# ngrabaskas/Torch-Automatic-Distributed-Neural-Network

Hardware: AMD Instinct MI355X
Metric: samples/sec whole-node ResNet-50 DP + GPT-2 PP at 1/2/4/8 MI355X; scaling eff (higher is better)
Workload: dtype bf16

## Files before the change

madnn/models/resnet.py:

```python
from __future__ import annotations

import os
from collections import namedtuple
from typing import List, Type

import torch
from torch import nn

from ..nn.conv import FusedConv2d
from ..nn.norm import FusedBatchNorm2d as BN
from ..nn.norm import FusedGlobalAvgPool2d, FusedMaxPool2d
from ..ops import (batch_norm_add_bn_relu, bn2_conv3_bn3_add_bn_relu, bn2_conv3_bn3_add_bn_relu_supported,
                   bn2_conv3_bn3_add_relu, bn2_conv3_bn3_supported, bn_relu_conv1x1,
                   bn_relu_conv1x1_epi_supported, bn_relu_conv3x3, bn_relu_conv3x3_supported, bn_relu_maxpool,
                   bn_relu_maxpool_supported, conv1x1_route, defer_res_mask)

_FORK_DS = os.environ.get("MADNN_FORK_DOWNSAMPLE", "1") != "0"
_DUAL_BN = os.environ.get("MADNN_DUAL_BN", "1") != "0"
_DS_SUB = os.environ.get("MADNN_DS_SUB", "1") != "0"


ROUTES = (IDENTITY_K9F, IDENTITY, DUAL_SUB, DUAL_K9F, DUAL, FORK_DS, PLAIN_DS) = (
    "identity+k9f", "identity", "dual+sub", "dual+k9f", "dual", "fork-ds", "plain-ds")
_Fused = namedtuple("_Fused", "bn1_conv2 bn2_conv3 bn3 dual")


def conv3x3(cin, cout, stride=1, groups=1, dilation=1):
    return FusedConv2d(cin, cout, 3, stride=stride, padding=dilation, groups=groups, bias=False, dilation=dilation)


def conv1x1(cin, cout, stride=1):
    return FusedConv2d(cin, cout, 1, stride=stride, bias=False)


class BasicBlock(nn.Module):
    expansion = 1

    def __init__(self, inplanes, planes, stride=1, downsample=None):
        super().__init__()
        self.conv1 = conv3x3(inplanes, planes, stride)
        self.bn1 = BN(planes)
        self.conv2 = conv3x3(planes, planes)
        self.bn2 = BN(planes)
        self.downsample = downsample

    def forward(self, x):
        idt = x if self.downsample is None else self.downsample(x)
        y, st = self.conv1(x, stats=True)
        out = self.bn1(y, relu=True, stats=st)
        y, st = self.conv2(out, stats=True)
        return self.bn2(y, residual=idt, relu=True, stats=st)


class Bottleneck(nn.Module):
    expansion = 4

    def __init__(self, inplanes, planes, stride=1, downsample=None):
        super().__init__()
        self.conv1 = conv1x1(inplanes, planes)
        self.bn1 = BN(planes)
        self.conv2 = conv3x3(planes, planes, stride)
        self.bn2 = BN(planes)
        self.conv3 = conv1x1(planes, planes * 4)
        self.bn3 = BN(planes * 4)
        self.downsample = downsample

    def forward(self, x):
        fused = self._fused()
        route = self._route(x, fused)
        ds = self.downsample
        if route in (IDENTITY_K9F, IDENTITY):
            y, st, side = self.conv1(x, stats=True, fork=True)
            if route == IDENTITY_K9F:
                defer_res_mask(side)
        elif route == PLAIN_DS:
            side = ds(x)
            y, st = self.conv1(x, stats=True)
        else:
            y, st, xf = self.conv1(x, stats=True, fork=2 if route == DUAL_SUB else True)
            if route == DUAL_K9F and not self._k9f_dual(y, xf):
                route = DUAL
            if route == FORK_DS:
                side = ds(xf)
            elif route == DUAL_SUB:
                side = ds[0].forward_subsampled(xf, stats=True)
            elif route == DUAL:
                side = ds[0](xf, stats=True)
        y1 = y
        y, st = self._bn1_conv2(y, st, fused)
        if route == IDENTITY_K9F and fused.bn2_conv3 and isinstance(y, torch.Tensor) and self.conv3._k9(y) \
                and bn2_conv3_bn3_supported(y, self.bn2, self.conv3.weight, self.bn3, side):
            return bn2_conv3_bn3_add_relu(y, self.bn2, self.conv3.weight, self.bn3, side, stats_in=st)
        if route == DUAL_K9F:
            if isinstance(y, torch.Tensor) and y.requires_grad \
                    and (y.shape, y.stride(), y.dtype) == (y1.shape, y1.stride(), y1.dtype):
                return bn2_conv3_bn3_add_bn_relu(y, self.bn2, self.conv3.weight, self.bn3, xf, ds[0].weight,
                                                 ds[1], stats_in=st)
            route, side = DUAL, ds[0](xf, stats=True)
        y, st = self._bn2_conv3(y, st, fused)
        if route in (DUAL_SUB, DUAL):
            return batch_norm_add_bn_relu(y, side[0], self.bn3, ds[1], st, side[1])
        return self.bn3(y, residual=side, relu=True, stats=st)

    def _fused(self) -> "_Fused":
        ds = self.downsample
        return _Fused(bn1_conv2=isinstance(self.bn1, BN) and isinstance(self.conv2, FusedConv2d),
                      bn2_conv3=isinstance(self.bn2, BN) and isinstance(self.conv3, FusedConv2d),
                      bn3=isinstance(self.bn3, BN),
                      dual=(isinstance(ds, nn.Sequential) and len(ds) == 2 and isinstance(ds[0], FusedConv2d)
                            and isinstance(ds[1], BN) and isinstance(self.bn3, BN)))

    def _dual_bn(self) -> bool:
        return _DUAL_BN and self._fused().dual

    def _route(self, x, fused: "_Fused") -> str:
        ds, tensor = self.downsample, isinstance(x, torch.Tensor)
        if ds is None:
            defer = (tensor and fused.bn3 and self.conv1._k9(x)
                     and conv1x1_route(x.size(1), self.conv1.weight.size(0))[1] == "k9")
            return IDENTITY_K9F if defer else IDENTITY
        if not _FORK_DS:
            return PLAIN_DS
        if not (_DUAL_BN and fused.dual):
            return FORK_DS
        if _DS_SUB and tensor and ds[0].subsampled_ok():
            return DUAL_SUB
        return DUAL_K9F if tensor and fused.bn2_conv3 and self.conv2.stride == (1, 1) else DUAL

    def _bn1_conv2(self, y, st, fused):
        if fused.bn1_conv2 and isinstance(y, torch.Tensor) and self.conv2._k13(y) \
                and bn_relu_conv3x3_supported(y, self.bn1, self.conv2.weight):
            return bn_relu_conv3x3(y, self.bn1, self.conv2.weight, stats_in=st, stats=True, checked=True)
        out = self.bn1(y, relu=True, stats=st)
        return self.conv2(out, stats=True)

    def _bn2_conv3(self, y, st, fused):
        if fused.bn2_conv3 and isinstance(y, torch.Tensor) and self.conv3._k9(y) \
                and bn_relu_conv1x1_epi_supported(y, self.bn2, self.conv3.weight):
            return bn_relu_conv1x1(y, self.bn2, self.conv3.weight, stats_in=st, stats=True, checked=True)
        out = self.bn2(y, relu=True, stats=st)
        return self.conv3(out, stats=True)

    def _k9f_dual(self, y1, xf) -> bool:
        ds = self.downsample
        return (isinstance(y1, torch.Tensor) and isinstance(xf, torch.Tensor) and self.conv3._k9(y1)
                and ds[0]._k9(xf) and bn2_conv3_bn3_add_bn_relu_supported(
                    y1, self.bn2, self.conv3.weight, self.bn3, xf, ds[0].weight, ds[1]))


class ResNet(nn.Module):
    def __init__(self, block: Type[nn.Module], layers: List[int], num_classes: int = 1000,
                 zero_init_residual: bool = True, width: int = 64):
        super().__init__()
        self.inplanes = width
        self.conv1 = FusedConv2d(3, width, 7, stride=2, padding=3, bias=False)
        self.bn1 = BN(width)
        self.maxpool = FusedMaxPool2d(3, stride=2, padding=1)
        self.layer1 = self._make_layer(block, width, layers[0])
        self.layer2 = self._make_layer(block, width * 2, layers[1], stride=2)
        self.layer3 = self._make_layer(block, width * 4, layers[2], stride=2)
        self.layer4 = self._make_layer(block, width * 8, layers[3], stride=2)
        self.avgpool = FusedGlobalAvgPool2d((1, 1))
        self.fc = nn.Linear(width * 8 * block.expansion, num_classes)
        for m in self.modules():
            if isinstance(m, nn.Conv2d):
                nn.init.kaiming_normal_(m.weight, mode="fan_out", nonlinearity="relu")
            elif isinstance(m, nn.BatchNorm2d):
                nn.init.ones_(m.weight)
                nn.init.zeros_(m.bias)
        if zero_init_residual:
            for m in self.modules():
                if isinstance(m, Bottleneck):
                    nn.init.zeros_(m.bn3.weight)
                elif isinstance(m, BasicBlock):
                    nn.init.zeros_(m.bn2.weight)

    def _make_layer(self, block, planes, blocks, stride=1):
        downsample = None
        if stride != 1 or self.inplanes != planes * block.expansion:
            downsample = nn.Sequential(conv1x1(self.inplanes, planes * block.expansion, stride),
                                       BN(planes * block.expansion))
        layers = [block(self.inplanes, planes, stride, downsample)]
        self.inplanes = planes * block.expansion
        layers += [block(self.inplanes, planes) for _ in range(1, blocks)]
        return nn.Sequential(*layers)

    def stem(self, x):
        y, st = self.conv1(x, stats=True)
        if isinstance(self.bn1, BN) and isinstance(self.maxpool, FusedMaxPool2d) \
                and bn_relu_maxpool_supported(y, self.bn1, self.maxpool):
            return bn_relu_maxpool(y, self.bn1, self.maxpool, st)
        return self.maxpool(self.bn1(y, relu=True, stats=st))

    def head(self, x):
        return self.fc(torch.flatten(self.avgpool(x), 1))

    def forward(self, x):
        x = self.layer4(self.layer3(self.layer2(self.layer1(self.stem(x)))))
        return self.head(x)

    def pipeline_layers(self):
        blocks = [b for layer in (self.layer1, self.layer2, self.layer3, self.layer4) for b in layer]
        return [_Bound(self, "stem"), *blocks, _Bound(self, "head")]


class _Bound(nn.Module):

    def __init__(self, model: nn.Module, method: str):
        super().__init__()
        self.parts = nn.ModuleDict({n: m for n, m in model.named_children()
                                    if n in {"stem": ("conv1", "bn1", "maxpool"),
                                             "head": ("avgpool", "fc")}[method]})
        object.__setattr__(self, "_model", model)
        self.method = method

    def forward(self, x):
        return getattr(self._model, self.method)(x)


def resnet18(num_classes: int = 1000, **kw) -> ResNet:
    return ResNet(BasicBlock, [2, 2, 2, 2], num_classes, **kw)


def resnet50(num_classes: int = 1000, **kw) -> ResNet:
    return ResNet(Bottleneck, [3, 4, 6, 3], num_classes, **kw)


def resnet101(num_classes: int = 1000, **kw) -> ResNet:
    return ResNet(Bottleneck, [3, 4, 23, 3], num_classes, **kw)
```

madnn/nn/conv.py:

```python
from __future__ import annotations

import os

import torch
from torch import nn

from .. import ops

_K9 = os.environ.get("MADNN_CONV1X1", "1") != "0"


class FusedConv2d(nn.Conv2d):
    def _k9(self, x: torch.Tensor) -> bool:
        return (_K9 and self.kernel_size == (1, 1) and self.stride == (1, 1) and self.dilation == (1, 1)
                and self.groups == 1 and self.bias is None and self.padding in ((0, 0), "valid")
                and ops.conv1x1_supported(x, self.weight))

    def _k13(self, x: torch.Tensor) -> bool:
        return (self.kernel_size == (3, 3) and self.stride == (1, 1) and self.padding == (1, 1)
                and self.dilation == (1, 1) and self.groups == 1 and self.bias is None
                and self.padding_mode == "zeros" and ops.conv3x3_supported(x, self.weight))

    def _k13s2(self, x: torch.Tensor) -> bool:
        return (self.kernel_size == (3, 3) and self.stride == (2, 2) and self.padding == (1, 1)
                and self.dilation == (1, 1) and self.groups == 1 and self.bias is None
                and self.padding_mode == "zeros" and ops.conv3x3_s2_supported(x, self.weight))

    def _k10(self, x: torch.Tensor) -> bool:
        return (self.kernel_size == (7, 7) and self.stride == (2, 2) and self.padding == (3, 3)
                and self.dilation == (1, 1) and self.groups == 1 and self.bias is None
                and ops.stem_supported(x, self.weight))

    def forward(self, x: torch.Tensor, stats: bool = False, fork: bool = False):
        if self._k9(x):
            return ops.conv1x1(x, self.weight, stats=stats, fork=fork)
        if not fork and self._k13(x):
            return ops.conv3x3(x, self.weight, stats=stats)
        if not fork and self._k13s2(x):
            return ops.conv3x3_s2(x, self.weight, stats=stats)
        if not fork and self._k10(x):
            return ops.stem_conv(x, self.weight, stats=stats)
        out = [super().forward(x)]
        if stats:
            out.append(None)
        if fork:
            out.append(x[:, :, ::2, ::2] if fork == 2 else x)
        return out[0] if len(out) == 1 else tuple(out)

    def subsampled_ok(self) -> bool:
        return (self.kernel_size == (1, 1) and self.stride == (2, 2) and self.padding in ((0, 0), "valid")
                and self.dilation == (1, 1) and self.groups == 1 and self.bias is None)

    def forward_subsampled(self, xs: torch.Tensor, stats: bool = False):
        if _K9 and ops.conv1x1_supported(xs, self.weight):
            return ops.conv1x1(xs, self.weight, stats=stats)
        y = torch.nn.functional.conv2d(xs, self.weight)
        return (y, None) if stats else y

    def extra_repr(self):
        k = {(1, 1): ", kernel=madnn.K9", (7, 7): ", kernel=madnn.K10",
             (3, 3): ", kernel=madnn.K13" if self.stride in ((1, 1), (2, 2)) else ""}.get(self.kernel_size, "")
        return super().extra_repr() + k
```

madnn/ops/__init__.py:

```python
from __future__ import annotations

import os
import threading
from pathlib import Path
from typing import Optional, Sequence

import torch
import torch.nn.functional as F

from . import reference

HERE = Path(__file__).resolve().parent
_KERNELS = HERE / "_madnn_kernels.so"
_lock = threading.Lock()
_loaded = {"kernels": False, "error": None}


def kernels_path() -> Path:
    return _KERNELS


class StaleKernelsError(RuntimeError):
    """The in-tree kernel library was built from different sources than the tree holds."""

# ... 714 lines not shown
        dout = _nhwc(dout.to(y.dtype))
        da, part = torch.ops.madnn.conv1x1_dgrad_bnb(dout, w, y, scale, shift)
        dw = _routed_conv1x1_wgrad(ctx.wgrad, dout, a, w)
        dy, dbw, dbb = torch.ops.madnn.bn_bwd_ext(da, y, bn_w, mean, invstd, scale, shift, part, True)
        need_bn = ctx.needs_input_grad[2] or ctx.needs_input_grad[3]
        return dy, dw, dbw if need_bn else None, dbb if need_bn else None, None, None, None


def bn_relu_conv1x1(y: torch.Tensor, bn, w: torch.Tensor, *, stats_in: Optional[torch.Tensor] = None,
                    stats: bool = False, checked: bool = False):
    if checked or bn_relu_conv1x1_epi_supported(y, bn, w):
        _need_native("bn_relu_conv1x1")
        return _with_stats(*_BNReluConv1x1EpiFn.apply(y, w, bn.weight, bn.bias, bn, stats_in, stats), stats)
    a = bn(y, relu=True, stats=stats_in) if _is_fused_bn(bn) else torch.relu(bn(y))
    if conv1x1_supported(a, w):
        return conv1x1(a, w, stats=stats)
    out = torch.nn.functional.conv2d(a, w.view(w.size(0), -1, 1, 1)) if a.dim() == 4 else torch.mm(
        a, w.reshape(w.size(0), -1).t())
    return (out, None) if stats else out


def bn_relu_conv1x1_epi_supported(y: torch.Tensor, bn, w: torch.Tensor) -> bool:
    return (_BN_DGRAD_EPI and isinstance(y, torch.Tensor) and _bn_trainable(bn)
            and conv1x1_supported(y, w) and bn_supported(y, bn.weight)
            and conv1x1_route(y.size(1), w.size(0))[1] == "k9")


def _k9f_head(y2, w3, bn2_w, bn2_b, bn2, stats_in):
    a2, mean2, invstd2, scale2, shift2, _ = _bn_fwd_train(y2, None, bn2_w, bn2_b, bn2, True, stats_in)
    y3, part = torch.ops.madnn.conv1x1_fwd(a2, w3, True)
    return a2, y3, part, (mean2, invstd2, scale2, shift2)


def _k9f_tail(ctx, da2, part, y2, bn2_w, bn2_stats, dw3, w3, dbw3, dbb3):
    dy2, dbw2, dbb2 = torch.ops.madnn.bn_bwd_ext(da2, y2, bn2_w, *bn2_stats, part, True)
    need2, need3 = (ctx.needs_input_grad[i] or ctx.needs_input_grad[i + 1] for i in (2, 4))
    return (dy2, dw3.to(w3.dtype).view(w3.shape), dbw2 if need2 else None, dbb2 if need2 else None,
            dbw3 if need3 else None, dbb3 if need3 else None)


class _BN2Conv3BN3Fn(torch.autograd.Function):

    @staticmethod
    def forward(ctx, y2, w3, bn2_w, bn2_b, bn3_w, bn3_b, idt, bn2, bn3, stats_in):
        a2, y3, part, bn2_stats = _k9f_head(y2, w3, bn2_w, bn2_b, bn2, stats_in)
        out, mean3, invstd3, scale3, shift3, mask = _bn_fwd_train(y3, idt, bn3_w, bn3_b, bn3, True, part)
        ctx.save_for_backward(y2, a2, w3, y3, mask, bn2_w, *bn2_stats, bn3_w, mean3, invstd3, scale3, shift3)
        return out

    @staticmethod
    def backward(ctx, dout):
        y2, a2, w3, y3, mask, bn2_w, *bn2_stats, bn3_w, mean3, invstd3, scale3, shift3 = ctx.saved_tensors
        dout = _like(dout, y3)
        coef, dbw3, dbb3 = torch.ops.madnn.bn_bwd_coef(dout, y3, mask, bn3_w, mean3, invstd3, scale3, shift3)
        da2, part, dw3 = torch.ops.madnn.bn3_conv3_bwd(dout, y3, mask, coef, w3, a2, y2, *bn2_stats[2:],
                                                       w3.dtype == torch.bfloat16)
        grads = _k9f_tail(ctx, da2, part, y2, bn2_w, bn2_stats, dw3, w3, dbw3, dbb3)
        dres = dout.view_as(dout)
        _attach(dres, "_madnn_resmask", mask)
        return (*grads, dres, None, None, None)


_BN3_CONV3_FUSED = os.environ.get("MADNN_BN3_CONV3_FUSED", "1") != "0"


def _k9f_supported(y2: torch.Tensor, bn2, w3: torch.Tensor, bn3, other: torch.Tensor) -> bool:
    return (_BN3_CONV3_FUSED and isinstance(y2, torch.Tensor) and isinstance(other, torch.Tensor)
            and bn_relu_conv1x1_epi_supported(y2, bn2, w3) and native_available()
            and bool(torch.ops.madnn.bn3_conv3_bwd_supported(y2.size(1), w3.size(0)))
            and conv1x1_route(y2.size(1), w3.size(0))[0] == "k9" and _bn_trainable(bn3)
            and bn3.weight.numel() == w3.size(0) and y2.requires_grad and torch.is_grad_enabled()
            and other.dtype == y2.dtype and other.dim() == y2.dim() and other.size(0) == y2.size(0)
            and other.shape[2:] == y2.shape[2:])


def bn2_conv3_bn3_supported(y2: torch.Tensor, bn2, w3: torch.Tensor, bn3, idt: torch.Tensor) -> bool:
    return (DEFER_RES_MASK and _k9f_supported(y2, bn2, w3, bn3, idt) and _res_mask_deferred(idt)
            and idt.size(1) == w3.size(0) and bn_supported(idt, bn3.weight))


def bn2_conv3_bn3_add_relu(y2: torch.Tensor, bn2, w3: torch.Tensor, bn3, idt: torch.Tensor,
                           stats_in: Optional[torch.Tensor] = None) -> torch.Tensor:
    _need_native("bn2_conv3_bn3_add_relu")
    return _BN2Conv3BN3Fn.apply(y2, w3, bn2.weight, bn2.bias, bn3.weight, bn3.bias, idt, bn2, bn3, stats_in)


class _BN2Conv3BN3DualFn(torch.autograd.Function):

    @staticmethod
    def forward(ctx, y2, w3, bn2_w, bn2_b, bn3_w, bn3_b, xf, w_ds, bnd_w, bnd_b, bn2, bn3, bn_ds, stats_in):
        a2, y3, part, bn2_stats = _k9f_head(y2, w3, bn2_w, bn2_b, bn2, stats_in)
        yd, part_d = torch.ops.madnn.conv1x1_fwd(xf, w_ds, True)
        out, mask, mean3, invstd3, _, _, mean_d, invstd_d, _, _ = torch.ops.madnn.bn_fwd_dual(
            y3, yd, bn3_w, bn3_b, bn3.running_mean, bn3.running_var, bn3.num_batches_tracked, float(bn3.momentum),
            float(bn3.eps), part, bnd_w, bnd_b, bn_ds.running_mean, bn_ds.running_var, bn_ds.num_batches_tracked,
            float(bn_ds.momentum), float(bn_ds.eps), part_d)
        ctx.save_for_backward(y2, a2, w3, y3, xf, w_ds, yd, mask, bn2_w, *bn2_stats, bn3_w, mean3, invstd3, bnd_w,
                              mean_d, invstd_d)
        return out

    @staticmethod
    def backward(ctx, dout):
        (y2, a2, w3, y3, xf, w_ds, yd, mask, bn2_w, *bn2_stats, bn3_w, mean3, invstd3, bnd_w, mean_d,
         invstd_d) = ctx.saved_tensors
        dout = _like(dout, y3)
        coef, dbw3, dbb3, dbwd, dbbd = torch.ops.madnn.bn_bwd_dual_coef(dout, y3, yd, mask, bn3_w, mean3, invstd3,
                                                                        bnd_w, mean_d, invstd_d)
        da2, part, dw3 = torch.ops.madnn.bn3_conv3_bwd(dout, y3, mask, coef[:3], w3, a2, y2, *bn2_stats[2:],
                                                       w3.dtype == torch.bfloat16)
        dxf, _, dwd = torch.ops.madnn.bn3_conv3_bwd(dout, yd, mask, coef[3:], w_ds, xf, None, None, None,
                                                    w_ds.dtype == torch.bfloat16)
        grads = _k9f_tail(ctx, da2, part, y2, bn2_w, bn2_stats, dw3, w3, dbw3, dbb3)
        needd = ctx.needs_input_grad[8] or ctx.needs_input_grad[9]
        return (*grads, dxf, dwd.to(w_ds.dtype).view(w_ds.shape), dbwd if needd else None,
                dbbd if needd else None, None, None, None, None)


_BN3_CONV3_DUAL = os.environ.get("MADNN_BN3_CONV3_DUAL", "1") != "0"


def bn2_conv3_bn3_add_bn_relu_supported(y2: torch.Tensor, bn2, w3: torch.Tensor, bn3, xf: torch.Tensor,
                                        w_ds: torch.Tensor, bn_ds) -> bool:
    return (_BN3_CONV3_DUAL and _k9f_supported(y2, bn2, w3, bn3, xf) and conv1x1_supported(xf, w_ds)
            and xf.size(1) == y2.size(1) and w_ds.size(0) == w3.size(0) and _bn_trainable(bn_ds)
            and bn_ds.weight.numel() == w3.size(0))


def bn2_conv3_bn3_add_bn_relu(y2: torch.Tensor, bn2, w3: torch.Tensor, bn3, xf: torch.Tensor, w_ds: torch.Tensor,
                              bn_ds, stats_in: Optional[torch.Tensor] = None) -> torch.Tensor:
    _need_native("bn2_conv3_bn3_add_bn_relu")
    return _BN2Conv3BN3DualFn.apply(y2, w3, bn2.weight, bn2.bias, bn3.weight, bn3.bias, xf, w_ds, bn_ds.weight,
                                    bn_ds.bias, bn2, bn3, bn_ds, stats_in)


class _BNReluMaxPoolFn(torch.autograd.Function):

    @staticmethod
    def forward(ctx, y, bn_w, bn_b, bn, stats_in, p):
        mean, invstd, scale, shift = torch.ops.madnn.bn_coef(y, bn_w, bn_b, bn.running_mean, bn.running_var,
                                                             bn.num_batches_tracked, float(bn.momentum),
                                                             float(bn.eps), stats_in)
        out, arg = torch.ops.madnn.pool_bn_fwd(y, scale, shift, int(p))
        ctx.save_for_backward(y, arg, bn_w, mean, invstd, scale, shift)
        ctx.p = int(p)
        return out

    @staticmethod
    def backward(ctx, dp):
        y, arg, bn_w, mean, invstd, scale, shift = ctx.saved_tensors
        dy, dw, db = torch.ops.madnn.pool_bn_bwd(dp, arg, y, bn_w, mean, invstd, scale, shift, ctx.p)
        return dy, dw, db, None, None, None


def bn_relu_maxpool_supported(y: torch.Tensor, bn, pool) -> bool:
    return (_POOL_BN and isinstance(y, torch.Tensor) and y.device.type == "cuda" and y.dtype == torch.bfloat16 and y.dim() == 4
            and y.is_contiguous(memory_format=torch.channels_last) and _bn_trainable(bn)
            and _pair(pool.kernel_size) == (3, 3) and _pair(pool.stride) == (2, 2)
            and _pair(pool.padding) in ((1, 1), (0, 0)) and _pair(pool.dilation) == (1, 1)
            and not pool.ceil_mode and not pool.return_indices
            and y.size(1) % 8 == 0 and 256 % (y.size(1) // 8) == 0 and y.numel() < 2 ** 31)


def bn_relu_maxpool(y: torch.Tensor, bn, pool, stats_in: Optional[torch.Tensor] = None):
    if bn_relu_maxpool_supported(y, bn, pool):
        _need_native("bn_relu_maxpool")
        p = pool.padding if isinstance(pool.padding, int) else pool.padding[0]
        return _BNReluMaxPoolFn.apply(y, bn.weight, bn.bias, bn, stats_in, p)
    a = bn(y, relu=True, stats=stats_in) if _is_fused_bn(bn) else torch.relu(bn(y))
    return pool(a)


_POOL_BN = os.environ.get("MADNN_POOL_BN", "1") != "0"


_K13 = os.environ.get("MADNN_CONV3X3", "1") != "0"
_K13_WGRAD = os.environ.get("MADNN_CONV3X3_WGRAD", "auto")


def _k13_halo_ok(W: int) -> bool:
    rb = 2 * 32
    rpi = 1024 // rb
    cap = ((255 // W) * W + 4 * W + rpi - 1) // rpi * rpi
    return max(cap * rb + rb + 2 * 64 * rb, 32 * 1024) <= 80 * 1024


def _k13_operands_ok(x: torch.Tensor, w: torch.Tensor) -> bool:
    if not _K13 or x.device.type != "cuda" or x.dtype != torch.bfloat16 or w.dtype != torch.bfloat16:
        return False
    if x.dim() != 4 or not x.is_contiguous(memory_format=torch.channels_last) or x.numel() == 0:
        return False
    if w.dim() != 4 or tuple(w.shape[1:]) != (x.size(1), 3, 3):
        return False
    return x.size(1) % 64 == 0 and w.size(0) % 64 == 0


def conv3x3_supported(x: torch.Tensor, w: torch.Tensor) -> bool:
    return _k13_operands_ok(x, w) and _k13_halo_ok(x.size(3))


def _flip3x3(w: torch.Tensor) -> torch.Tensor:
    return w.flip(2, 3).transpose(0, 1).contiguous(memory_format=torch.channels_last)


def _conv3x3_wgrad(dy: torch.Tensor, x: torch.Tensor, w: torch.Tensor) -> torch.Tensor:
    k13 = lambda: torch.ops.madnn.conv3x3_wgrad(dy, x, w.dtype == torch.bfloat16)
    lib = lambda: torch.ops.aten.convolution_backward(
        dy, x, w, None, (1, 1), (1, 1), (1, 1), False, (0, 0), 1, (False, True, False))[1]
    if _K13_WGRAD == "k13":
        dw = k13()
    elif _K13_WGRAD == "miopen" or (_K13_WGRAD == "wide" and x.size(3) < 48):
        dw = lib()
    elif _K13_WGRAD == "wide":
        dw = k13()
    else:
        dw = tuned_wgrad(("conv3x3",) + tuple(x.shape) + (w.size(0),), lib, k13)
    return _like(dw, w)


class _Conv3x3Fn(torch.autograd.Function):

    @staticmethod
    def forward(ctx, x, w, stats):
        y, part = torch.ops.madnn.conv3x3_fwd(x, _nhwc(w), bool(stats))
        ctx.save_for_backward(x, w)
        ctx.mark_non_differentiable(part)
        return y, part

    @staticmethod
    def backward(ctx, dy, _dpart):
        x, w = ctx.saved_tensors
        dy = _nhwc(dy.to(x.dtype))
        dx = dw = None
        if ctx.needs_input_grad[0]:
            dx = torch.ops.madnn.conv3x3_fwd(dy, _flip3x3(w), False)[0]
        if ctx.needs_input_grad[1]:
            dw = _conv3x3_wgrad(dy, x, w)
        return dx, dw, None


class _BNReluConv3x3Fn(torch.autograd.Function):

    @staticmethod
    def forward(ctx, y, w, bn_w, bn_b, bn, stats_in, want_stats):
        a, mean, invstd, scale, shift, _ = _bn_fwd_train(y, None, bn_w, bn_b, bn, True, stats_in)
        out, part = torch.ops.madnn.conv3x3_fwd(a, _nhwc(w), bool(want_stats))
        ctx.save_for_backward(y, a, w, bn_w, mean, invstd, scale, shift)
        ctx.mark_non_differentiable(part)
        return out, part

    @staticmethod
    def backward(ctx, dout, _dpart):
        y, a, w, bn_w, mean, invstd, scale, shift = ctx.saved_tensors
        dout = _nhwc(dout.to(y.dtype))
        da, part = torch.ops.madnn.conv3x3_fwd_bnb(dout, _flip3x3(w), y, scale, shift)
        dw = _conv3x3_wgrad(dout, a, w)
        dy, dbw, dbb = torch.ops.madnn.bn_bwd_ext(da, y, bn_w, mean, invstd, scale, shift, part, True)
        need_bn = ctx.needs_input_grad[2] or ctx.needs_input_grad[3]
        return dy, dw, dbw if need_bn else None, dbb if need_bn else None, None, None, None


def bn_relu_conv3x3_supported(y: torch.Tensor, bn, w: torch.Tensor) -> bool:
    return (_BN_DGRAD_EPI and isinstance(y, torch.Tensor) and _bn_trainable(bn) and conv3x3_supported(y, w)
            and y.size(1) == w.size(1) and bn_supported(y, bn.weight))


def bn_relu_conv3x3(y: torch.Tensor, bn, w: torch.Tensor, *, stats_in: Optional[torch.Tensor] = None,
                    stats: bool = False, checked: bool = False):
    if checked or bn_relu_conv3x3_supported(y, bn, w):
        _need_native("bn_relu_conv3x3")
        return _with_stats(*_BNReluConv3x3Fn.apply(y, w, bn.weight, bn.bias, bn, stats_in, stats), stats)
    a = bn(y, relu=True, stats=stats_in) if _is_fused_bn(bn) else torch.relu(bn(y))
    if conv3x3_supported(a, w):
        return conv3x3(a, w, stats=stats)
    out = torch.nn.functional.conv2d(a, w, padding=1)
    return (out, None) if stats else out


_BN_DGRAD_EPI = os.environ.get("MADNN_BN_DGRAD_EPI", "1") != "0"


def conv3x3(x: torch.Tensor, w: torch.Tensor, *, stats: bool = False):
    _need_native("conv3x3")
    y, part = _Conv3x3Fn.apply(x, w, stats)
    return (y, part) if stats else y


_K13_S2_MAX_W = int(os.environ.get("MADNN_CONV3X3_S2_MAX_W", "16"))


def conv3x3_s2_supported(x: torch.Tensor, w: torch.Tensor) -> bool:
    return (_k13_operands_ok(x, w) and x.size(2) % 2 == 0 and x.size(3) % 2 == 0
            and 2 <= x.size(3) <= _K13_S2_MAX_W and x.size(2) <= 4 * _K13_S2_MAX_W)


class _Conv3x3S2Fn(torch.autograd.Function):

    @staticmethod
    def forward(ctx, x, w, stats):
        y, part = torch.ops.madnn.conv3x3_fwd_s2(x, _nhwc(w), bool(stats))
        ctx.save_for_backward(x, w)
        ctx.mark_non_differentiable(part)
        return y, part

    @staticmethod
    def backward(ctx, dy, _dpart):
        x, w = ctx.saved_tensors
        dy = _nhwc(dy.to(x.dtype))
        dx, dw, _ = torch.ops.aten.convolution_backward(dy, x, w, None, (2, 2), (1, 1), (1, 1), False, (0, 0), 1,
                                                        (ctx.needs_input_grad[0], ctx.needs_input_grad[1], False))
        return dx, dw, None


def conv3x3_s2(x: torch.Tensor, w: torch.Tensor, *, stats: bool = False):
    _need_native("conv3x3_s2")
    y, part = _Conv3x3S2Fn.apply(x, w, stats)
    return (y, part) if stats else y


_K10 = os.environ.get("MADNN_STEM", "1") != "0"


def stem_supported(x: torch.Tensor, w: torch.Tensor) -> bool:
    if not _K10 or x.device.type != "cuda" or x.dtype != torch.bfloat16 or w.dtype != torch.bfloat16:
        return False
    if x.dim() != 4 or x.size(1) != 3 or tuple(w.shape) != (64, 3, 7, 7) or x.numel() == 0:
        return False
    H, W = x.size(2), x.size(3)
    return (x.is_contiguous(memory_format=torch.channels_last) and H >= 7 and W >= 8 and W % 8 == 0
            and (W - 1) // 2 + 1 <= 128 and 7 * (3 * W // 8) <= 1024)


def _stem_pack(w: torch.Tensor) -> torch.Tensor:
    wp = w.new_zeros((64, 7, 8, 4))
    wp[:, :, :7, :3] = w.permute(0, 2, 3, 1)
    return wp


class _StemFn(torch.autograd.Function):

    @staticmethod
    def forward(ctx, x, w, stats):
        y, part = torch.ops.madnn.stem_fwd(x, _stem_pack(w), bool(stats))
        ctx.save_for_backward(x, w)
        ctx.mark_non_differentiable(part)
        return y, part

    @staticmethod
    def backward(ctx, dy, _dpart):
        x, w = ctx.saved_tensors
        dy = _nhwc(dy.to(x.dtype))
        dx = dw = None
        if ctx.needs_input_grad[0]:
            dx = torch.ops.aten.convolution_backward(dy, x, w, None, (2, 2), (3, 3), (1, 1), False, (0, 0), 1,
                                                     (True, False, False))[0]
        if ctx.needs_input_grad[1]:
            dw = _like(torch.ops.madnn.stem_wgrad(dy, x).to(w.dtype), w)
        return dx, dw, None


def stem_conv(x: torch.Tensor, w: torch.Tensor, *, stats: bool = False):
    _need_native("stem_conv")
    y, part = _StemFn.apply(x, w, stats)
    return (y, part) if stats else y


def hidden_supported(h: int) -> bool:
    return h % 8 == 0 and h <= 16384


FUSED_LINEAR = os.environ.get("MADNN_FUSED_LINEAR", "1") != "0"

def _gelu_tanh_grad(p: torch.Tensor) -> torch.Tensor:
    k0, k1 = 0.7978845608028654, 0.044715
    t = torch.tanh(k0 * (p + k1 * p * p * p))
    return 0.5 * (1 + t) + 0.5 * p * (1 - t * t) * k0 * (1 + 3 * k1 * p * p)


GELU_KIND = {"tanh": 1, "none": 2}


def _gelu_grad_ref(p: torch.Tensor, kind: int) -> torch.Tensor:
    if kind == 1:
        return _gelu_tanh_grad(p)
    cdf = 0.5 * (1.0 + torch.erf(p * 0.7071067811865476))
    return cdf + p * torch.exp(-0.5 * p * p) * 0.3989422804014327


def bias_grad(dy: torch.Tensor, pre: Optional[torch.Tensor] = None, bias_dtype: Optional[torch.dtype] = None,
              kind: int = 1):
    bias_dtype = bias_dtype or dy.dtype
    n = dy.shape[-1]
    if not _is_dev(dy) or n % 8:
        acc = torch.promote_types(dy.dtype, torch.float32)
        g = dy.to(acc)
        if pre is not None:
            g = g * _gelu_grad_ref(pre.to(acc), kind)
        return g.reshape(-1, n).sum(0).to(bias_dtype), (g.to(dy.dtype) if pre is not None else None)
    db, dp = _need_native("bias_grad").bias_grad(dy, pre, bias_dtype, kind)
    return db, (dp.view(dy.shape) if pre is not None else None)


GELU_KERNEL = os.environ.get("MADNN_GELU_KERNEL", "1") != "0"


def gelu_tanh(x: torch.Tensor, kind: int = 1) -> torch.Tensor:
    if GELU_KERNEL and _is_dev(x) and x.numel() % 8 == 0 and x.dtype in (torch.bfloat16, torch.float32):
        return _need_native("gelu_tanh").gelu_fwd(x, kind)
    return F.gelu(x, approximate="tanh" if kind == 1 else "none")


def grad_sink(weight: torch.Tensor) -> Optional[torch.Tensor]:
    space = getattr(weight, "_madnn_space", None)
    if space is None or weight.grad is not None:
        return None
    return space.grad_slot(weight)


WGRAD = os.environ.get("MADNN_WGRAD", "auto")

_CHOICES: dict = {"wgrad": {}, "gelu_fwd": {}, "dgelu": {}, "dgrad": {}}
_WGRAD_CHOICE, _GELU_FWD_CHOICE, _DGELU_CHOICE, _DGRAD_CHOICE = _CHOICES.values()
_TUNE = {"timed": 0, "table": None}
_TUNE_MS: dict = {}

TUNE_TABLE = os.path.join(os.path.dirname(os.path.dirname(os.path.abspath(__file__))), "tuning",
                          "choices_gfx950.json")


def load_tuning_table(path: Optional[str] = None) -> int:
    import ast
    import json

    if os.environ.get("MADNN_TUNE_TABLE", "1") == "0":
        return 0
    path = path or os.environ.get("MADNN_TUNE_TABLE_PATH") or TUNE_TABLE
    try:
        with open(path) as f:
            data = json.load(f)
    except (OSError, ValueError):
        return 0
    n = 0
    for name, dst in _CHOICES.items():
        for k, v in data.get(name, {}).items():
            dst.setdefault(ast.literal_eval(k), v)
            n += 1
    _TUNE["table"] = path
    return n


def export_choices(path: str) -> None:
    import json

    data = {"arch": "gfx950"}
    for name, table in _CHOICES.items():
        data[name] = {repr(k): v for k, v in sorted(table.items(), key=repr)}
    with open(path, "w") as f:
        json.dump(data, f, indent=1)
        f.write("\n")


def sync_choices(group=None, src: int = 0) -> None:
    import torch.distributed as dist

    if not dist.is_initialized() or dist.get_world_size(group) <= 1:
        return
    obj = [_CHOICES]
    dist.broadcast_object_list(obj, src=src, group=group)
    for name, table in obj[0].items():
        _CHOICES[name].update(table)


def tuning_timings() -> int:
    return _TUNE["timed"]


def tuning_measurements() -> list:
    return [{"table": tab, "key": repr(key), "ms": {k: round(v, 4) for k, v in ms.items()},
             "chosen": _CHOICES[tab].get(key)} for (tab, key), ms in _TUNE_MS.items()]


def _wgrad_k12_ok(g2, x2, out) -> bool:
    return (_is_dev(g2) and g2.dtype == x2.dtype == out.dtype == torch.bfloat16 and g2.shape[0] % 64 == 0
            and g2.shape[1] % 8 == 0 and x2.shape[1] % 8 == 0 and g2.is_contiguous() and x2.is_contiguous()
            and out.is_contiguous() and load_kernels())


def _time_wgrad(fn, iters: int = 3) -> float:
    fn()
    s, e = torch.cuda.Event(enable_timing=True), torch.cuda.Event(enable_timing=True)
    s.record()
    for _ in range(iters):
        fn()
    e.record()
    e.synchronize()
    return s.elapsed_time(e)


def _timed_choice(table_name: str, key, cands: dict, default: str) -> str:
    table = _CHOICES[table_name]
    choice = table.get(key)
    if choice in cands:
        return choice
    if torch.cuda.is_current_stream_capturing():
        return default
    _TUNE["timed"] += 1
    times = _TUNE_MS[(table_name, key)] = {k: _time_wgrad(f) for k, f in cands.items()}
    choice = table[key] = min(times, key=times.get)
    return choice


def wgrad_into(g2: torch.Tensor, x2: torch.Tensor, out: torch.Tensor) -> torch.Tensor:
    lib = lambda: torch.mm(g2.t(), x2, out=out)
    if WGRAD == "lt" or not _wgrad_k12_ok(g2, x2, out):
        return lib()
    return tuned_wgrad(("linear",) + tuple(g2.shape) + (x2.shape[1],), lib,
                       lambda: torch.ops.madnn.linear_wgrad(g2, x2, out, False, 0),
# ... 210 lines not shown
    @staticmethod
    def backward(ctx, g):
        x, weight, *pre = ctx.saved_tensors
        db = None
        g_out = g
        if ctx.gelu:
            db, g = bias_grad(g, pre[0], ctx.bias_dtype or g.dtype)
            if ctx.bias_dtype is None:
                db = None
        elif ctx.bias_dtype is not None and ctx.needs_input_grad[2]:
            db = _out_bias_grad(g, ctx.bias_dtype)
        g2 = g.reshape(-1, g.shape[-1])
        dx = dw = None
        if ctx.needs_input_grad[0]:
            dx = dgrad(g2, weight).view(*x.shape[:-1], weight.shape[1])
        if ctx.needs_input_grad[1]:
            dw = _weight_grad(g2, x.reshape(-1, x.shape[-1]), ctx.param)
        ctx.param = None
        return dx, dw, db, None, (g_out if ctx.has_res else None)


def _linear_residual_fwd(a: torch.Tensor, weight, bias, residual):
    out = _lt_epilogue(a, weight, bias, residual, False)
    if out is not None:
        return out[0]
    y = F.linear(a, weight, bias if bias is None or bias.dtype == a.dtype else bias.to(a.dtype))
    return y + residual if residual is not None else y


_LT_KN_FAILED = []


def _dgrad_plus(g2: torch.Tensor, weight: torch.Tensor, res2: torch.Tensor) -> torch.Tensor:
    if not _LT_KN_FAILED and _lt_ok(g2, weight, False, True) and g2.is_contiguous():
        try:
            y, _ = _need_native("lt_linear").lt_linear(g2, weight, None, res2.contiguous().to(g2.dtype), False, False,
                                                       True)
            return y
        except RuntimeError as e:
            _LT_KN_FAILED.append(e)
    return torch.addmm(res2.to(g2.dtype), g2, weight)


class _LinearTeeFn(torch.autograd.Function):

    @staticmethod
    def forward(ctx, x, weight, bias):
        ctx.bias_dtype = bias.dtype if bias is not None else None
        ctx.param = weight
        ctx.save_for_backward(x, weight)
        return _linear_residual_fwd(x, weight, bias, None), x.view_as(x)

    @staticmethod
    def backward(ctx, g, gx):
        x, weight = ctx.saved_tensors
        db = None
        if ctx.bias_dtype is not None and ctx.needs_input_grad[2]:
            db = _out_bias_grad(g, ctx.bias_dtype)
        g2 = g.reshape(-1, g.shape[-1])
        dx = dw = None
        if ctx.needs_input_grad[0]:
            if gx is None:
                dx = g2 @ weight
            else:
                dx = _dgrad_plus(g2, weight, gx.reshape(-1, weight.shape[1]))
            dx = dx.view(*x.shape[:-1], weight.shape[1])
        if ctx.needs_input_grad[1]:
            dw = _weight_grad(g2, x.reshape(-1, x.shape[-1]), ctx.param)
        ctx.param = None
        return dx, dw, db


def linear_tee(x: torch.Tensor, weight: torch.Tensor, bias: Optional[torch.Tensor] = None):
    if not torch.is_grad_enabled() or not _is_dev(x) or weight.shape[0] % 8:
        return F.linear(x, weight, bias if bias is None or bias.dtype == x.dtype else bias.to(x.dtype)), x
    return _LinearTeeFn.apply(x, weight, bias)


class _GeluMLPFn(torch.autograd.Function):

    @staticmethod
    def forward(ctx, x, w1, b1, w2, b2, residual, kind=1):
        a, pre = _gelu_linear_fwd(x, w1, b1, kind)
        ctx.kind = kind
        y = _linear_residual_fwd(a, w2, b2, residual)
        ctx.save_for_backward(x, w1, pre, a, w2)
        ctx.b1_dtype = b1.dtype if b1 is not None else None
        ctx.b2_dtype = b2.dtype if b2 is not None else None
        ctx.bias_dtype = ctx.b2_dtype
        ctx.params = (w1, w2)
        ctx.has_res = residual is not None
        ctx.res_is_x = residual is x
        return y

    @staticmethod
    def backward(ctx, g):
        x, w1, pre, a, w2 = ctx.saved_tensors
        p1, p2 = ctx.params
        ctx.params = None
        need = ctx.needs_input_grad
        db2 = _out_bias_grad(g, ctx.b2_dtype) if ctx.b2_dtype is not None and need[4] else None
        g2 = g.reshape(-1, g.shape[-1])
        if not g2.is_contiguous():
            g2 = g2.contiguous()
        a2 = a.reshape(-1, a.shape[-1])
        dw2 = _weight_grad(g2, a2, p2) if need[3] else None
        dh, db1 = dgrad_dgelu(g2, w2, pre.reshape(-1, pre.shape[-1]), ctx.b1_dtype or g2.dtype, ctx.kind)
        if ctx.b1_dtype is None or not need[2]:
            db1 = None
        x2 = x.reshape(-1, x.shape[-1])
        dw1 = _weight_grad(dh, x2, p1) if need[1] else None
        if ctx.res_is_x and need[0]:
            dx = _dgrad_plus(dh, w1, g2).view(*x.shape[:-1], w1.shape[1])
            return dx, dw1, db1, dw2, db2, None, None
        dx = (dh @ w1).view(*x.shape[:-1], w1.shape[1]) if need[0] else None
        return dx, dw1, db1, dw2, db2, (g if ctx.has_res else None), None


def gelu_mlp(x: torch.Tensor, w1: torch.Tensor, b1: Optional[torch.Tensor], w2: torch.Tensor,
             b2: Optional[torch.Tensor], residual: Optional[torch.Tensor] = None,
             approximate: str = "tanh") -> torch.Tensor:
    if residual is not None and residual.shape[:-1] != x.shape[:-1]:
        raise ValueError("gelu_mlp: residual must have the output's shape")
    if approximate not in GELU_KIND:
        raise ValueError(f"gelu_mlp: approximate must be 'tanh' or 'none', not {approximate!r}")
    if not _is_dev(x) or not torch.is_grad_enabled() or w1.shape[0] % 8 or w2.shape[0] % 8:
        h = F.gelu(F.linear(x, w1, b1), approximate=approximate)
        y = F.linear(h, w2, b2)
        return y + residual if residual is not None else y
    return _GeluMLPFn.apply(x, w1, b1, w2, b2, residual, GELU_KIND[approximate])


def linear(x: torch.Tensor, weight: torch.Tensor, bias: Optional[torch.Tensor] = None, gelu: bool = False,
           force_fn: bool = False, residual: Optional[torch.Tensor] = None):
    if residual is not None and residual.shape[:-1] != x.shape[:-1]:
        raise ValueError("linear: residual must have the output's shape")
    if not torch.is_grad_enabled() or (not force_fn and (not _is_dev(x) or weight.shape[0] % 8)):
        if not torch.is_grad_enabled() and _is_dev(x) and (gelu or residual is not None) and weight.shape[0] % 8 == 0:
            out = _lt_epilogue(x, weight, bias, residual, gelu)
            if out is not None:
                return out[0]
        y = F.linear(x, weight, bias)
        y = F.gelu(y, approximate="tanh") if gelu else y
        return y + residual if residual is not None else y
    return _LinearFn.apply(x, weight, bias, gelu, residual)


__all__ = [
    "bucket_pack", "bucket_unpack", "flat_scale_cast", "sgd_step", "adam_step", "grad_norm", "layer_norm",
    "rms_norm", "batch_norm_act", "bn_supported", "cross_entropy", "attention", "attention_qkvpacked", "attention_supported",
    "max_pool2d", "max_pool_supported", "conv1x1", "conv1x1_route", "batch_norm_add_bn_relu",
    "batch_norm_dual_supported", "bn_relu_conv1x1", "bn_relu_maxpool",
    "bn_relu_maxpool_supported", "bn_relu_conv3x3", "bn_relu_conv3x3_supported",
    "bn_relu_conv1x1_epi_supported", "bn2_conv3_bn3_add_relu", "bn2_conv3_bn3_supported", "bn2_conv3_bn3_add_bn_relu", "bn2_conv3_bn3_add_bn_relu_supported", "conv1x1_supported", "stem_conv", "stem_supported", "native_available", "load_kernels", "kernels_path", "hidden_supported", "reference",
    "linear", "linear_tee", "gelu_mlp", "bias_grad", "gelu_tanh", "grad_sink", "wgrad_into", "tuned_wgrad", "dgrad",
    "dgrad_dgelu", "load_tuning_table", "export_choices", "sync_choices", "tuning_timings", "tuning_measurements",
]

if os.environ.get("MADNN_EAGER_LOAD", "0") == "1":
    load_kernels()

load_tuning_table()
```

madnn/ops/csrc/binding.cpp:

```cpp
#include <torch/library.h>
#include <ATen/ATen.h>
#include <ATen/hip/impl/HIPGuardImplMasqueradingAsCUDA.h>
#include <ATen/hip/impl/HIPStreamMasqueradingAsCUDA.h>
#include <hip/hip_runtime.h>

#include <vector>

#include "attn.h"

extern "C" {
hipError_t madnn_bucket_pack(void* const*, const int64_t*, const int64_t*, int, void*, int, int, float, hipStream_t);
hipError_t madnn_bucket_unpack(void* const*, const int64_t*, const int64_t*, int, void*, int, int, float, hipStream_t);
hipError_t madnn_flat_scale_cast(const void*, void*, int64_t, int, int, float, hipStream_t);
hipError_t madnn_sgd_step(float*, const void*, int, float*, void*, int, int64_t, float, float, float, float, int, int,
                          float, const float*, hipStream_t);
hipError_t madnn_adam_step(float*, const void*, int, float*, float*, void*, int, int64_t, float, float, float, float,
                           float, int, float, float, float, const float*, hipStream_t);
int madnn_sqnorm_grid(int64_t);
hipError_t madnn_sqnorm_partial(const void*, int, int64_t, float, float*, int, hipStream_t);
hipError_t madnn_norm_finalize(const float*, int, float, float*, hipStream_t);
hipError_t madnn_norm_fwd(const void*, const void*, const void*, const void*, void*, void*, float*, float*, int64_t,
                          int, float, int, int, int, hipStream_t);
int64_t madnn_norm_bwd_workspace(int64_t, int);
hipError_t madnn_norm_bwd(const void*, const void*, const void*, const float*, const float*, const void*, void*, void*,
                          void*, void*, int, float*, int64_t, int, int, int, int, hipStream_t);
int madnn_bn_supported(int);
int madnn_bn_partial_rows(int64_t, int);
hipError_t madnn_bn_fwd(const void*, const void*, void*, unsigned char*, int64_t, int, int, int, int, float, float,
                        const float*, const float*, float*, float*, int64_t*, float*, float*, float*, float*, float*,
                        const float*, int, hipStream_t);
int madnn_bias_grad_supported(int64_t, int);
int madnn_bias_grad_rows(int64_t, int, int);
hipError_t madnn_bias_grad(const void*, const void*, void*, int64_t, int, int, float*, void*, int, int, hipStream_t);
hipError_t madnn_gelu_fwd(const void*, void*, int64_t, int, int, hipStream_t);
hipError_t madnn_rope_qkv(const void*, void*, const float*, const float*, int64_t, int, int, int, int, int, hipStream_t);
hipError_t madnn_swiglu_fwd(const void*, void*, int64_t, int, hipStream_t);
hipError_t madnn_swiglu_bwd(const void*, const void*, void*, int64_t, int, hipStream_t);
int madnn_attn_supported(int);
hipError_t madnn_attn_fwd(const MadnnAttnArgs*, int, int, hipStream_t);
hipError_t madnn_attn_bwd(const MadnnAttnArgs*, int, int, hipStream_t);
int64_t madnn_attn_colsum_rows(int, int);
hipError_t madnn_attn_colsum_finalize(const float*, int64_t, int64_t, void*, int, hipStream_t);
int madnn_maxpool_supported(int64_t, int, int);
hipError_t madnn_maxpool_fwd(const void*, void*, void*, int, int, int, int, int, int, int, int, int, int, hipStream_t);
int madnn_pool_bn_supported(int64_t, int);
int madnn_pool_bn_bwd_rows(int64_t, int);
hipError_t madnn_pool_bn_fwd(const void*, const float*, const float*, void*, void*, int, int, int, int, int, int, int,
                             hipStream_t);
hipError_t madnn_pool_bn_bwd(const void*, const void*, const void*, const float*, const float*, const float*,
                             const float*, const float*, void*, float*, float*, float*, float*, int, int, int, int, int,
                             int, int, hipStream_t);
hipError_t madnn_maxpool_bwd(const void*, const void*, void*, int, int, int, int, int, int, int, int, int, int,
                             hipStream_t);
hipError_t madnn_xent_fwd(const void*, int, const int64_t*, int64_t, int64_t, int64_t, int, int, float*, float*,
                          hipStream_t);
hipError_t madnn_xent_bwd(const void*, int, const int64_t*, const float*, int64_t, int64_t, int64_t, int, int, int64_t,
                          const float*, void*, hipStream_t);
int madnn_xent_fused_chunks(int64_t);
hipError_t madnn_xent_fused(const void*, int, const int64_t*, int64_t, int64_t, int64_t, int, int, int64_t,
                            const float*, float*, void*, hipStream_t);
hipError_t madnn_xent_rescale(void*, int, int64_t, const float*, hipStream_t);
hipError_t madnn_bn_bwd(const void*, const void*, const unsigned char*, int, void*, void*, int64_t, int, int, int,
                        const float*, const float*, const float*, const float*, const float*, float*, float*, float*,
                        float*, hipStream_t);
hipError_t madnn_bn_fwd_dual(const void*, const void*, void*, unsigned char*, int64_t, int, float, float, const float*,
                             const float*, float*, float*, int64_t*, float*, float*, float*, float*, const float*, int,
                             float, float, const float*, const float*, float*, float*, int64_t*, float*, float*,
                             float*, float*, const float*, int, float*, hipStream_t);
hipError_t madnn_bn_bwd_dual(const void*, const void*, const void*, const unsigned char*, void*, void*, int64_t, int,
                             const float*, const float*, const float*, const float*, const float*, const float*,
                             float*, float*, float*, float*, float*, float*, hipStream_t);
hipError_t madnn_bn_bwd_dual_coef(const void*, const void*, const void*, const unsigned char*, int64_t, int,
                                  const float*, const float*, const float*, const float*, const float*, const float*,
                                  float*, float*, float*, float*, float*, float*, hipStream_t);
hipError_t madnn_bn_bwd_coef(const void*, const void*, const unsigned char*, int, int64_t, int, int, int, const float*,
                             const float*, const float*, const float*, const float*, float*, float*, float*, float*,
                             hipStream_t);
int madnn_bn3_conv3_bwd_supported(int64_t, int64_t);
int madnn_bn3_conv3_bwd_groups(int64_t);
hipError_t madnn_bn3_conv3_bwd(const void*, const void*, const unsigned char*, const float*, const void*, const void*,
                               const void*, const float*, const float*, void*, float*, float*, void*, int, int64_t,
                               int64_t, int64_t, hipStream_t);
int madnn_conv1x1_supported(int64_t, int64_t);
int madnn_conv1x1_stat_rows(int64_t, int64_t, int64_t);
hipError_t madnn_conv1x1_fwd(const void*, const void*, void*, float*, int64_t, int64_t, int64_t, hipStream_t);
hipError_t madnn_conv1x1_dgrad(const void*, const void*, void*, const void*, int64_t, int64_t, int64_t, const void*,
                               const float*, const float*, float*, hipStream_t, const unsigned char* = nullptr);
int madnn_conv1x1_dgrad_rows(int64_t, int64_t, int64_t);
int64_t madnn_conv1x1_wgrad_ws(int64_t, int64_t, int64_t);
hipError_t madnn_conv1x1_wgrad(const void*, const void*, void*, int, float*, int64_t, int64_t, int64_t, hipStream_t);
hipError_t madnn_bn_coef(const void*, int64_t, int, float, float, const float*, const float*, float*, float*, int64_t*,
                         float*, float*, float*, float*, float*, const float*, int, hipStream_t);
int madnn_stem_supported(int, int);
int madnn_stem_stat_rows(int, int, int);
hipError_t madnn_stem_fwd(const void*, const void*, void*, float*, int, int, int, hipStream_t);
int64_t madnn_stem_wgrad_ws(int, int, int);
hipError_t madnn_stem_wgrad(const void*, const void*, float*, float*, int, int, int, hipStream_t);
int madnn_gemm_supported(int64_t, int64_t, int64_t, int64_t, int64_t);
int madnn_conv3x3_supported(int, int, int, int);
int madnn_conv3x3_stat_rows(int64_t);
hipError_t madnn_conv3x3_fwd(const void*, const void*, void*, float*, int, int, int, int, int, hipStream_t);
int madnn_conv3x3_s2_supported(int, int, int, int);
int madnn_conv3x3_s2_stat_rows(int, int, int);
hipError_t madnn_conv3x3_fwd_s2(const void*, const void*, void*, float*, int, int, int, int, int, hipStream_t);
int64_t madnn_conv3x3_wgrad_ws(int, int, int, int, int);
hipError_t madnn_conv3x3_fwd_bnb(const void*, const void*, void*, float*, const void*, const float*, const float*, int,
                                 int, int, int, int, hipStream_t);
hipError_t madnn_bn_bwd_ext(const void*, const void*, void*, int64_t, int, int, const float*, const float*,
                            const float*, const float*, const float*, float*, float*, float*, const float*, int, float*,
                            hipStream_t);
int madnn_bn_prereduce_floats(int);
hipError_t madnn_conv3x3_wgrad(const void*, const void*, float*, void*, int, int, int, int, int, int, hipStream_t);
hipError_t madnn_linear_fwd(const void*, const void*, const void*, int, const void*, void*, void*, int, int64_t,
                            int64_t, int64_t, hipStream_t);
hipError_t madnn_linear_dgrad(const void*, const void*, const void*, void*, int64_t, int64_t, int64_t, hipStream_t);
int madnn_wgrad_splits(int64_t, int64_t, int64_t);
hipError_t madnn_linear_wgrad4h(const void*, const void*, void*, float*, int, int, int64_t, int64_t, int64_t,
                                hipStream_t);
hipError_t madnn_linear_wgrad4(const void*, const void*, void*, float*, int, int, int64_t, int64_t, int64_t,
                               hipStream_t);
hipError_t madnn_linear_wgrad(const void*, const void*, void*, float*, int, int, int64_t, int64_t, int64_t,
                              hipStream_t);
int madnn_gemmp_supported(int64_t, int64_t, int64_t, int);
hipError_t madnn_linear_fwd_p(const void*, const void*, const void*, int, void*, void*, int, int64_t, int64_t,
                              int64_t, hipStream_t);
hipError_t madnn_linear_dgrad_p(const void*, const void*, const void*, void*, float*, int64_t, int64_t, int64_t, int,
                                hipStream_t);
hipError_t madnn_colsum_finalize(const float*, int, int64_t, void*, int, hipStream_t);
hipError_t madnn_hwq_wait(const int*, int, int64_t, int*, hipStream_t);
hipError_t madnn_hwq_set(int*, int, hipStream_t);
hipError_t madnn_hwq_batch(const int*, const int*, int, int*, int*, int, int64_t, int*, const int*, hipStream_t);
hipError_t madnn_hwq_spin(int64_t, hipStream_t);
}

namespace {

int dt_code(const at::Tensor& t) {
  switch (t.scalar_type()) {
    case at::kFloat: return 0;
    case at::kBFloat16: return 1;
    case at::kHalf: return 2;
    default: TORCH_CHECK(false, "madnn: unsupported dtype ", t.scalar_type());
  }
  return -1;
}

hipStream_t cur_stream(const at::Tensor& t) {
  return at::hip::getCurrentHIPStreamMasqueradingAsCUDA(t.device().index()).stream();
}

void check(hipError_t e, const char* what) {
  TORCH_CHECK(e == hipSuccess, "madnn HIP kernel ", what, " failed: ", hipGetErrorString(e));
}

void check_dev(const at::Tensor& t, const char* name) {
  TORCH_CHECK(t.is_cuda(), "madnn: ", name, " must be a HIP device tensor");
}

void check_dense(const at::Tensor& t) {
  TORCH_CHECK(t.is_non_overlapping_and_dense(), "madnn bucket op: tensor must be non-overlapping and dense");
}

void bucket_copy(bool pack, at::TensorList tensors, const at::Tensor& flat, at::IntArrayRef offsets, double scale) {
  check_dev(flat, "flat");
  TORCH_CHECK(flat.is_contiguous(), "flat bucket must be contiguous");
  TORCH_CHECK(tensors.size() == offsets.size(), "tensors/offsets length mismatch");
  if (tensors.empty()) return;
  at::hip::HIPGuardMasqueradingAsCUDA guard(flat.device());
  const int tdt = dt_code(tensors[0]);
  std::vector<void*> ptrs;
  std::vector<int64_t> numels, offs;
  ptrs.reserve(tensors.size());
  for (size_t i = 0; i < tensors.size(); ++i) {
    const auto& t = tensors[i];
    check_dev(t, "bucket tensor");
    check_dense(t);
    TORCH_CHECK(dt_code(t) == tdt, "bucket tensors must share one dtype");
    TORCH_CHECK(offsets[i] >= 0 && offsets[i] + t.numel() <= flat.numel(), "bucket offset out of range");
    ptrs.push_back(t.data_ptr());
    numels.push_back(t.numel());
    offs.push_back(offsets[i]);
  }
  auto fn = pack ? madnn_bucket_pack : madnn_bucket_unpack;
  check(fn(ptrs.data(), offs.data(), numels.data(), (int)ptrs.size(), flat.data_ptr(), tdt, dt_code(flat),
           (float)scale, cur_stream(flat)),
        pack ? "bucket_pack" : "bucket_unpack");
}

void bucket_pack(at::TensorList srcs, at::Tensor flat, at::IntArrayRef offsets, double scale) {
  bucket_copy(true, srcs, flat, offsets, scale);
}

void bucket_unpack(at::TensorList dsts, at::Tensor flat, at::IntArrayRef offsets, double scale) {
  bucket_copy(false, dsts, flat, offsets, scale);
}

void flat_scale_cast(const at::Tensor& src, at::Tensor dst, double scale) {
  check_dev(src, "src");
  check_dev(dst, "dst");
  TORCH_CHECK(src.is_contiguous() && dst.is_contiguous(), "flat_scale_cast needs contiguous tensors");
  TORCH_CHECK(src.numel() == dst.numel(), "flat_scale_cast size mismatch");
  at::hip::HIPGuardMasqueradingAsCUDA guard(src.device());
  check(madnn_flat_scale_cast(src.data_ptr(), dst.data_ptr(), src.numel(), dt_code(src), dt_code(dst), (float)scale,
                              cur_stream(src)),
        "flat_scale_cast");
}

const float* opt_scale(const c10::optional<at::Tensor>& s) {
  if (!s.has_value()) return nullptr;
  TORCH_CHECK(s->scalar_type() == at::kFloat && s->is_cuda(), "device scale must be a float HIP tensor");
  return s->data_ptr<float>();
}

void sgd_step(at::Tensor master, const at::Tensor& grad, const c10::optional<at::Tensor>& mom,
              const c10::optional<at::Tensor>& model, double lr, double momentum, double dampening,
              double weight_decay, bool nesterov, bool first_step, double grad_scale,
              const c10::optional<at::Tensor>& dscale) {
  check_dev(master, "master");
  TORCH_CHECK(master.scalar_type() == at::kFloat && master.is_contiguous(), "master must be contiguous fp32");
  TORCH_CHECK(grad.is_contiguous() && grad.numel() == master.numel(), "grad must be contiguous and match master");
  if (momentum != 0.0) TORCH_CHECK(mom.has_value() && mom->numel() == master.numel(), "momentum buffer required");
  if (model.has_value()) TORCH_CHECK(model->is_contiguous() && model->numel() == master.numel(), "model copy size");
  at::hip::HIPGuardMasqueradingAsCUDA guard(master.device());
  check(madnn_sgd_step(master.data_ptr<float>(), grad.data_ptr(), dt_code(grad),
                       mom.has_value() ? mom->data_ptr<float>() : nullptr,
                       model.has_value() ? model->data_ptr() : nullptr, model.has_value() ? dt_code(*model) : -1,
                       master.numel(), (float)lr, (float)momentum, (float)dampening, (float)weight_decay,
                       nesterov ? 1 : 0, first_step ? 1 : 0, (float)grad_scale, opt_scale(dscale),
                       cur_stream(master)),
        "sgd_step");
}

void adam_step(at::Tensor master, const at::Tensor& grad, at::Tensor m1, at::Tensor m2,
               const c10::optional<at::Tensor>& model, double lr, double beta1, double beta2, double eps,
               double weight_decay, bool adamw, int64_t step, double grad_scale,
               const c10::optional<at::Tensor>& dscale) {
  check_dev(master, "master");
  TORCH_CHECK(master.scalar_type() == at::kFloat && master.is_contiguous(), "master must be contiguous fp32");
  TORCH_CHECK(grad.is_contiguous() && grad.numel() == master.numel(), "grad must be contiguous and match master");
  TORCH_CHECK(m1.numel() == master.numel() && m2.numel() == master.numel(), "adam state size");
  if (model.has_value()) TORCH_CHECK(model->is_contiguous() && model->numel() == master.numel(), "model copy size");
  TORCH_CHECK(step >= 1, "adam step must be >= 1");
  at::hip::HIPGuardMasqueradingAsCUDA guard(master.device());
  const double bc1 = 1.0 - std::pow(beta1, (double)step);
  const double bc2 = 1.0 - std::pow(beta2, (double)step);
  check(madnn_adam_step(master.data_ptr<float>(), grad.data_ptr(), dt_code(grad), m1.data_ptr<float>(),
                        m2.data_ptr<float>(), model.has_value() ? model->data_ptr() : nullptr,
                        model.has_value() ? dt_code(*model) : -1, master.numel(), (float)lr, (float)beta1,
                        (float)beta2, (float)eps, (float)weight_decay, adamw ? 1 : 0, (float)bc1,
                        (float)std::sqrt(bc2), (float)grad_scale, opt_scale(dscale), cur_stream(master)),
// ... 654 lines not shown
                                cur_stream(dy)),
          "colsum_finalize");
  return {dx, db};
}

void conv3_check(const at::Tensor& x, const at::Tensor& w, const char* op) {
  check_dev(x, "x");
  check_dev(w, "w");
  TORCH_CHECK(x.scalar_type() == at::kBFloat16 && w.scalar_type() == at::kBFloat16, op, ": bf16 only");
  TORCH_CHECK(x.dim() == 4 && x.is_contiguous(at::MemoryFormat::ChannelsLast), op, ": x must be NHWC 4-D");
  TORCH_CHECK(w.dim() == 4 && w.size(2) == 3 && w.size(3) == 3 && w.size(1) == x.size(1) &&
                  w.is_contiguous(at::MemoryFormat::ChannelsLast),
              op, ": w must be a channels_last [Co, Ci, 3, 3]");
}

std::tuple<at::Tensor, at::Tensor> conv3x3_fwd_s2(const at::Tensor& x, const at::Tensor& w, bool stats) {
  conv3_check(x, w, "conv3x3_s2");
  const int N = (int)x.size(0), Ci = (int)x.size(1), H = (int)x.size(2), W = (int)x.size(3), Co = (int)w.size(0);
  TORCH_CHECK(madnn_conv3x3_s2_supported(H, W, Ci, Co), "conv3x3_s2: unsupported shape Ci=", Ci, " Co=", Co, " H=", H,
              " W=", W);
  at::hip::HIPGuardMasqueradingAsCUDA guard(x.device());
  at::Tensor y = at::empty({N, Co, H / 2, W / 2}, x.options().memory_format(at::MemoryFormat::ChannelsLast));
  const int64_t rows = stats ? madnn_conv3x3_s2_stat_rows(N, H, W) : 0;
  at::Tensor part = at::empty({rows, 2, Co}, x.options().dtype(at::kFloat));
  check(madnn_conv3x3_fwd_s2(x.data_ptr(), w.data_ptr(), y.data_ptr(), stats ? part.data_ptr<float>() : nullptr, N,
                             H, W, Ci, Co, cur_stream(x)),
        "conv3x3_fwd_s2");
  return {y, part};
}

std::tuple<at::Tensor, at::Tensor> conv3x3_fwd(const at::Tensor& x, const at::Tensor& w, bool stats) {
  conv3_check(x, w, "conv3x3");
  const int N = (int)x.size(0), Ci = (int)x.size(1), H = (int)x.size(2), W = (int)x.size(3), Co = (int)w.size(0);
  TORCH_CHECK(madnn_conv3x3_supported(H, W, Ci, Co), "conv3x3: unsupported shape Ci=", Ci, " Co=", Co, " W=", W);
  at::hip::HIPGuardMasqueradingAsCUDA guard(x.device());
  at::Tensor y = at::empty({N, Co, H, W}, x.options().memory_format(at::MemoryFormat::ChannelsLast));
  const int64_t rows = stats ? madnn_conv3x3_stat_rows((int64_t)N * H * W) : 0;
  at::Tensor part = at::empty({rows, 2, Co}, x.options().dtype(at::kFloat));
  check(madnn_conv3x3_fwd(x.data_ptr(), w.data_ptr(), y.data_ptr(), stats ? part.data_ptr<float>() : nullptr, N, H,
                          W, Ci, Co, cur_stream(x)),
        "conv3x3_fwd");
  return {y, part};
}

std::tuple<at::Tensor, at::Tensor> conv3x3_fwd_bnb(const at::Tensor& x, const at::Tensor& w, const at::Tensor& bny,
                                                   const at::Tensor& scale, const at::Tensor& shift) {
  conv3_check(x, w, "conv3x3");
  check_dev(bny, "bny");
  TORCH_CHECK(bny.scalar_type() == at::kBFloat16, "conv3x3: bf16 only");
  const int N = (int)x.size(0), Ci = (int)x.size(1), H = (int)x.size(2), W = (int)x.size(3), Co = (int)w.size(0);
  TORCH_CHECK(bny.dim() == 4 && bny.size(0) == N && bny.size(1) == Co && bny.size(2) == H && bny.size(3) == W &&
                  bny.is_contiguous(at::MemoryFormat::ChannelsLast),
              "conv3x3_fwd_bnb: bny must be the NHWC [N, Co, H, W] BN input");
  const float* sc = vec_ptr(scale, Co, "conv3x3_fwd_bnb", "scale");
  const float* sh = vec_ptr(shift, Co, "conv3x3_fwd_bnb", "shift");
  TORCH_CHECK(madnn_conv3x3_supported(H, W, Ci, Co), "conv3x3: unsupported shape Ci=", Ci, " Co=", Co, " W=", W);
  at::hip::HIPGuardMasqueradingAsCUDA guard(x.device());
  at::Tensor y = at::empty({N, Co, H, W}, x.options().memory_format(at::MemoryFormat::ChannelsLast));
  at::Tensor part = at::empty({madnn_conv3x3_stat_rows((int64_t)N * H * W), 2, Co}, x.options().dtype(at::kFloat));
  check(madnn_conv3x3_fwd_bnb(x.data_ptr(), w.data_ptr(), y.data_ptr(), part.data_ptr<float>(), bny.data_ptr(), sc, sh,
                              N, H, W, Ci, Co, cur_stream(x)),
        "conv3x3_fwd_bnb");
  return {y, part};
}

std::tuple<at::Tensor, at::Tensor, at::Tensor> bn_bwd_ext(const at::Tensor& dy, const at::Tensor& x,
                                                          const c10::optional<at::Tensor>& w,
                                                          const at::Tensor& save_mean, const at::Tensor& save_invstd,
                                                          const at::Tensor& scale, const at::Tensor& shift,
                                                          const at::Tensor& partial, bool relu) {
  check_dev(x, "x");
  const int64_t C = x.size(1);
  const int64_t M = bn_rows(x, C);
  TORCH_CHECK(x.scalar_type() == at::kBFloat16 && dy.scalar_type() == at::kBFloat16 && dy.strides() == x.strides(),
              "bn_bwd_ext: bf16 dy / x of one layout");
  TORCH_CHECK(partial.scalar_type() == at::kFloat && partial.is_contiguous() && partial.dim() == 3 &&
                  partial.size(1) == 2 && partial.size(2) == C,
              "bn_bwd_ext: partial must be fp32 [rows, 2, C]");
  at::hip::HIPGuardMasqueradingAsCUDA guard(x.device());
  auto fo = x.options().dtype(at::kFloat);
  at::Tensor dx = at::empty_like(x), dw = at::empty({C}, fo), db = at::empty({C}, fo), coef = at::empty({3 * C}, fo);
  at::Tensor ws = at::empty({(int64_t)madnn_bn_prereduce_floats((int)C)}, fo);
  check(madnn_bn_bwd_ext(dy.data_ptr(), x.data_ptr(), dx.data_ptr(), M, (int)C, relu ? 1 : 0, optf(w),
                         save_mean.data_ptr<float>(), save_invstd.data_ptr<float>(), scale.data_ptr<float>(),
                         shift.data_ptr<float>(), dw.data_ptr<float>(), db.data_ptr<float>(), coef.data_ptr<float>(),
                         partial.data_ptr<float>(), (int)partial.size(0), ws.data_ptr<float>(), cur_stream(x)),
        "bn_bwd_ext");
  return {dx, dw, db};
}

at::Tensor conv3x3_wgrad(const at::Tensor& dy, const at::Tensor& x, bool out_bf16) {
  check_dev(x, "x");
  check_dev(dy, "dy");
  TORCH_CHECK(x.scalar_type() == at::kBFloat16 && dy.scalar_type() == at::kBFloat16, "conv3x3_wgrad: bf16 only");
  TORCH_CHECK(x.dim() == 4 && x.is_contiguous(at::MemoryFormat::ChannelsLast) && dy.dim() == 4 &&
                  dy.is_contiguous(at::MemoryFormat::ChannelsLast),
              "conv3x3_wgrad: NHWC 4-D tensors");
  TORCH_CHECK(dy.size(0) == x.size(0) && dy.size(2) == x.size(2) && dy.size(3) == x.size(3), "conv3x3_wgrad: shapes");
  const int N = (int)x.size(0), Ci = (int)x.size(1), H = (int)x.size(2), W = (int)x.size(3), Co = (int)dy.size(1);
  const int64_t nws = madnn_conv3x3_wgrad_ws(N, H, W, Ci, Co);
  TORCH_CHECK(nws > 0, "conv3x3_wgrad: unsupported shape Ci=", Ci, " Co=", Co, " H=", H, " W=", W);
  at::hip::HIPGuardMasqueradingAsCUDA guard(x.device());
  at::Tensor ws = at::empty({nws}, x.options().dtype(at::kFloat));
  at::Tensor dw = at::empty({Co, Ci, 3, 3},
                            x.options().dtype(out_bf16 ? at::kBFloat16 : at::kFloat).memory_format(at::MemoryFormat::ChannelsLast));
  check(madnn_conv3x3_wgrad(dy.data_ptr(), x.data_ptr(), ws.data_ptr<float>(), dw.data_ptr(), out_bf16 ? 1 : 0, N, H, W,
                            Ci, Co, cur_stream(x)),
        "conv3x3_wgrad");
  return dw;
}

void stem_check_x(const at::Tensor& x) {
  check_dev(x, "x");
  TORCH_CHECK(x.scalar_type() == at::kBFloat16 && x.dim() == 4 && x.size(1) == 3, "stem: x must be bf16 [N, 3, H, W]");
  TORCH_CHECK(x.is_contiguous(at::MemoryFormat::ChannelsLast), "stem: x must be channels_last");
  TORCH_CHECK(madnn_stem_supported((int)x.size(2), (int)x.size(3)), "stem: unsupported image size ", x.size(2), "x",
              x.size(3));
}

std::tuple<at::Tensor, at::Tensor> stem_fwd(const at::Tensor& x, const at::Tensor& wp, bool stats) {
  stem_check_x(x);
  check_dev(wp, "wp");
  TORCH_CHECK(wp.scalar_type() == at::kBFloat16 && wp.is_contiguous() && wp.numel() == 64 * 224,
              "stem: packed weight must be contiguous bf16 [64, 7, 8, 4]");
  const int N = (int)x.size(0), H = (int)x.size(2), W = (int)x.size(3);
  const int64_t Ho = (H - 1) / 2 + 1, Wo = (W - 1) / 2 + 1;
  at::hip::HIPGuardMasqueradingAsCUDA guard(x.device());
  at::Tensor y = at::empty({N, 64, Ho, Wo}, x.options().memory_format(at::MemoryFormat::ChannelsLast));
  const int64_t rows = stats ? madnn_stem_stat_rows(N, H, W) : 0;
  at::Tensor part = at::empty({rows, 2, 64}, x.options().dtype(at::kFloat));
  check(madnn_stem_fwd(x.data_ptr(), wp.data_ptr(), y.data_ptr(), stats ? part.data_ptr<float>() : nullptr, N, H, W,
                       cur_stream(x)),
        "stem_fwd");
  return {y, part};
}

at::Tensor stem_wgrad(const at::Tensor& dy, const at::Tensor& x) {
  stem_check_x(x);
  check_dev(dy, "dy");
  const int N = (int)x.size(0), H = (int)x.size(2), W = (int)x.size(3);
  TORCH_CHECK(dy.scalar_type() == at::kBFloat16 && dy.dim() == 4 && dy.size(0) == N && dy.size(1) == 64 &&
                  dy.size(2) == (H - 1) / 2 + 1 && dy.size(3) == (W - 1) / 2 + 1,
              "stem_wgrad: dy must be bf16 [N, 64, Ho, Wo]");
  TORCH_CHECK(dy.is_contiguous(at::MemoryFormat::ChannelsLast), "stem_wgrad: dy must be channels_last");
  at::hip::HIPGuardMasqueradingAsCUDA guard(x.device());
  at::Tensor ws = at::empty({madnn_stem_wgrad_ws(N, H, W)}, x.options().dtype(at::kFloat));
  at::Tensor dw = at::empty({64, 3, 7, 7}, x.options().dtype(at::kFloat));
  check(madnn_stem_wgrad(x.data_ptr(), dy.data_ptr(), ws.data_ptr<float>(), dw.data_ptr<float>(), N, H, W,
                         cur_stream(x)),
        "stem_wgrad");
  return dw;
}

struct XentGeom {
  int64_t n_rows_all, n_loss_rows, seq, ld;
};

XentGeom xent_geom(const at::Tensor& logits, const at::Tensor& targets, bool shift) {
  TORCH_CHECK(logits.is_contiguous(), "xent: logits must be contiguous");
  TORCH_CHECK(targets.scalar_type() == at::kLong && targets.is_contiguous(), "xent: int64 contiguous targets");
  XentGeom g;
  g.ld = logits.size(-1);
  g.n_rows_all = logits.numel() / g.ld;
  TORCH_CHECK(targets.numel() == g.n_rows_all, "xent: one target per logit row");
  if (shift) {
    TORCH_CHECK(logits.dim() == 3, "xent shift mode needs [B, S, V] logits");
    g.seq = logits.size(1);
    g.n_loss_rows = logits.size(0) * (g.seq - 1);
  } else {
    g.seq = 0;
    g.n_loss_rows = g.n_rows_all;
  }
  return g;
}

std::tuple<at::Tensor, at::Tensor> xent_fwd(const at::Tensor& logits, const at::Tensor& targets, bool shift,
                                            int64_t V, int64_t ignore_index) {
  check_dev(logits, "logits");
  const XentGeom g = xent_geom(logits, targets, shift);
  TORCH_CHECK(V > 0 && V <= g.ld, "xent: bad vocabulary size");
  at::hip::HIPGuardMasqueradingAsCUDA guard(logits.device());
  auto fo = logits.options().dtype(at::kFloat);
  at::Tensor loss = at::empty({g.n_loss_rows}, fo), lse = at::empty({g.n_loss_rows}, fo);
  check(madnn_xent_fwd(logits.data_ptr(), dt_code(logits), targets.data_ptr<int64_t>(), g.n_loss_rows, g.seq, g.ld,
                       (int)V, (int)ignore_index, loss.data_ptr<float>(), lse.data_ptr<float>(), cur_stream(logits)),
        "xent_fwd");
  return {loss, lse};
}

at::Tensor xent_bwd(const at::Tensor& logits, const at::Tensor& targets, const at::Tensor& lse, bool shift, int64_t V,
                    int64_t ignore_index, const at::Tensor& gscale) {
  check_dev(logits, "logits");
  const XentGeom g = xent_geom(logits, targets, shift);
  TORCH_CHECK(gscale.scalar_type() == at::kFloat && gscale.is_cuda(), "xent: fp32 device grad scale");
  at::hip::HIPGuardMasqueradingAsCUDA guard(logits.device());
  at::Tensor grad = at::empty_like(logits);
  check(madnn_xent_bwd(logits.data_ptr(), dt_code(logits), targets.data_ptr<int64_t>(), lse.data_ptr<float>(),
                       g.n_loss_rows, g.seq, g.ld, (int)V, (int)ignore_index, g.n_rows_all, gscale.data_ptr<float>(),
                       grad.data_ptr(), cur_stream(logits)),
        "xent_bwd");
  return grad;
}

bool xent_fused_ok(const at::Tensor& logits) {
  return (logits.scalar_type() == at::kBFloat16 || logits.scalar_type() == at::kHalf) && logits.is_contiguous() &&
         madnn_xent_fused_chunks(logits.size(-1)) > 0 && (reinterpret_cast<uintptr_t>(logits.data_ptr()) & 15) == 0;
}

std::tuple<at::Tensor, at::Tensor> xent_fused(const at::Tensor& logits, const at::Tensor& targets, bool shift,
                                              int64_t V, int64_t ignore_index, const at::Tensor& gscale) {
  check_dev(logits, "logits");
  const XentGeom g = xent_geom(logits, targets, shift);
  TORCH_CHECK(V > 0 && V <= g.ld, "xent: bad vocabulary size");
  TORCH_CHECK(xent_fused_ok(logits), "xent_fused: 16-bit contiguous logits with 16-byte aligned rows");
  TORCH_CHECK(gscale.scalar_type() == at::kFloat && gscale.is_cuda(), "xent: fp32 device grad scale");
  at::hip::HIPGuardMasqueradingAsCUDA guard(logits.device());
  at::Tensor loss = at::empty({g.n_loss_rows}, logits.options().dtype(at::kFloat));
  at::Tensor grad = at::empty_like(logits);
  check(madnn_xent_fused(logits.data_ptr(), dt_code(logits), targets.data_ptr<int64_t>(), g.n_loss_rows, g.seq, g.ld,
                         (int)V, (int)ignore_index, g.n_rows_all, gscale.data_ptr<float>(), loss.data_ptr<float>(),
                         grad.data_ptr(), cur_stream(logits)),
        "xent_fused");
  return {loss, grad};
}

void xent_rescale(at::Tensor grad, const at::Tensor& g) {
  check_dev(grad, "grad");
  TORCH_CHECK(grad.is_contiguous() && g.scalar_type() == at::kFloat && g.is_cuda(), "xent_rescale: bad operands");
  at::hip::HIPGuardMasqueradingAsCUDA guard(grad.device());
  check(madnn_xent_rescale(grad.data_ptr(), dt_code(grad), grad.numel(), g.data_ptr<float>(), cur_stream(grad)),
        "xent_rescale");
}

std::tuple<at::Tensor, at::Tensor> maxpool_fwd(const at::Tensor& x, int64_t k, int64_t s, int64_t p, bool need_arg) {
  check_dev(x, "x");
  TORCH_CHECK(x.dim() == 4 && x.is_contiguous(at::MemoryFormat::ChannelsLast), "maxpool: NHWC 4-D input");
  const int64_t N = x.size(0), C = x.size(1), H = x.size(2), W = x.size(3);
  TORCH_CHECK(madnn_maxpool_supported(x.numel(), (int)C, (int)k), "maxpool: unsupported shape");
  TORCH_CHECK(k > 0 && s > 0 && p >= 0 && 2 * p <= k, "maxpool: bad window");
  const int64_t Ho = (H + 2 * p - k) / s + 1, Wo = (W + 2 * p - k) / s + 1;
  TORCH_CHECK(Ho > 0 && Wo > 0, "maxpool: empty output");
  at::hip::HIPGuardMasqueradingAsCUDA guard(x.device());
  at::Tensor y = at::empty({N, C, Ho, Wo}, x.options().memory_format(at::MemoryFormat::ChannelsLast));
  at::Tensor arg = at::empty({need_arg ? N * Ho * Wo * C : 0}, x.options().dtype(at::kByte));
  check(madnn_maxpool_fwd(x.data_ptr(), y.data_ptr(), need_arg ? arg.data_ptr() : nullptr, (int)N, (int)H, (int)W,
                          (int)C, (int)Ho, (int)Wo, (int)k, (int)s, (int)p, dt_code(x), cur_stream(x)),
        "maxpool_fwd");
  return {y, arg};
}

at::Tensor maxpool_bwd(const at::Tensor& dy, const at::Tensor& arg, int64_t H, int64_t W, int64_t k, int64_t s,
                       int64_t p) {
  check_dev(dy, "dy");
  TORCH_CHECK(dy.dim() == 4, "maxpool_bwd: 4-D grad");
  const int64_t N = dy.size(0), C = dy.size(1), Ho = dy.size(2), Wo = dy.size(3);
  TORCH_CHECK(arg.numel() == dy.numel() && arg.scalar_type() == at::kByte, "maxpool_bwd: argmax map mismatch");
  TORCH_CHECK(Ho == (H + 2 * p - k) / s + 1 && Wo == (W + 2 * p - k) / s + 1, "maxpool_bwd: geometry mismatch");
  at::Tensor dyc = dy.contiguous(at::MemoryFormat::ChannelsLast);
  at::hip::HIPGuardMasqueradingAsCUDA guard(dy.device());
  at::Tensor dx = at::empty({N, C, H, W}, dy.options().memory_format(at::MemoryFormat::ChannelsLast));
  TORCH_CHECK(madnn_maxpool_supported(dx.numel(), (int)C, (int)k), "maxpool_bwd: unsupported shape");
  check(madnn_maxpool_bwd(dyc.data_ptr(), arg.data_ptr(), dx.data_ptr(), (int)N, (int)H, (int)W, (int)C, (int)Ho,
                          (int)Wo, (int)k, (int)s, (int)p, dt_code(dy), cur_stream(dy)),
        "maxpool_bwd");
  return dx;
}

std::tuple<at::Tensor, at::Tensor> pool_bn_fwd(const at::Tensor& y, const at::Tensor& scale, const at::Tensor& shift,
                                               int64_t p) {
  check_dev(y, "y");
  TORCH_CHECK(y.dim() == 4 && y.is_contiguous(at::MemoryFormat::ChannelsLast) && y.scalar_type() == at::kBFloat16,
              "pool_bn: bf16 NHWC 4-D input");
  const int64_t N = y.size(0), C = y.size(1), H = y.size(2), W = y.size(3);
  TORCH_CHECK(madnn_pool_bn_supported(y.numel(), (int)C) && p >= 0 && p <= 1, "pool_bn: unsupported shape");
  TORCH_CHECK(scale.numel() == C && shift.numel() == C && scale.scalar_type() == at::kFloat &&
                  shift.scalar_type() == at::kFloat && scale.is_contiguous() && shift.is_contiguous(),
              "pool_bn: fp32 [C] scale/shift");
  const int64_t Ho = (H + 2 * p - 3) / 2 + 1, Wo = (W + 2 * p - 3) / 2 + 1;
  TORCH_CHECK(Ho > 0 && Wo > 0, "pool_bn: empty output");
  at::hip::HIPGuardMasqueradingAsCUDA guard(y.device());
  at::Tensor out = at::empty({N, C, Ho, Wo}, y.options().memory_format(at::MemoryFormat::ChannelsLast));
  at::Tensor arg = at::empty({N * Ho * Wo * C}, y.options().dtype(at::kByte));
  check(madnn_pool_bn_fwd(y.data_ptr(), scale.data_ptr<float>(), shift.data_ptr<float>(), out.data_ptr(),
                          arg.data_ptr(), (int)N, (int)H, (int)W, (int)C, (int)Ho, (int)Wo, (int)p, cur_stream(y)),
        "pool_bn_fwd");
  return {out, arg};
}

std::tuple<at::Tensor, at::Tensor, at::Tensor> pool_bn_bwd(const at::Tensor& dp, const at::Tensor& arg,
                                                           const at::Tensor& y, const c10::optional<at::Tensor>& w,
                                                           const at::Tensor& mean, const at::Tensor& invstd,
                                                           const at::Tensor& scale, const at::Tensor& shift,
                                                           int64_t p) {
  check_dev(y, "y");
  const int64_t N = y.size(0), C = y.size(1), H = y.size(2), W = y.size(3);
  const int64_t Ho = (H + 2 * p - 3) / 2 + 1, Wo = (W + 2 * p - 3) / 2 + 1;
  TORCH_CHECK(dp.dim() == 4 && dp.size(0) == N && dp.size(1) == C && dp.size(2) == Ho && dp.size(3) == Wo,
              "pool_bn_bwd: gradient shape");
  TORCH_CHECK(arg.numel() == dp.numel() && arg.scalar_type() == at::kByte, "pool_bn_bwd: argmax map mismatch");
  at::Tensor dpc = dp.to(at::kBFloat16).contiguous(at::MemoryFormat::ChannelsLast);
  at::hip::HIPGuardMasqueradingAsCUDA guard(y.device());
  auto fo = y.options().dtype(at::kFloat);
  at::Tensor dy = at::empty_like(y);
  at::Tensor dw = at::empty({C}, fo), db = at::empty({C}, fo), coef = at::empty({3 * C}, fo);
  at::Tensor ws = at::empty({(int64_t)madnn_pool_bn_bwd_rows(N * H * W, (int)C) * 2 * C}, fo);
  check(madnn_pool_bn_bwd(dpc.data_ptr(), arg.data_ptr(), y.data_ptr(), optf(w), mean.data_ptr<float>(),
                          invstd.data_ptr<float>(), scale.data_ptr<float>(), shift.data_ptr<float>(), dy.data_ptr(),
                          dw.data_ptr<float>(), db.data_ptr<float>(), coef.data_ptr<float>(), ws.data_ptr<float>(),
                          (int)N, (int)H, (int)W, (int)C, (int)Ho, (int)Wo, (int)p, cur_stream(y)),
        "pool_bn_bwd");
  return {dy, dw, db};
}

std::tuple<at::Tensor, at::Tensor> bias_grad(const at::Tensor& dy, const c10::optional<at::Tensor>& pre,
                                             at::ScalarType bias_dtype, int64_t gelu_kind) {
  TORCH_CHECK(gelu_kind == 1 || gelu_kind == 2, "bias_grad: gelu_kind 1 (tanh) or 2 (erf)");
  check_dev(dy, "dy");
  at::Tensor g = dy.contiguous();
  const int64_t N = g.size(-1), M = g.numel() / N;
  TORCH_CHECK(madnn_bias_grad_supported(M, (int)N), "bias_grad: last dim must be a multiple of 8");
  at::Tensor pc, dp;
  if (pre.has_value()) {
    pc = pre->contiguous();
    TORCH_CHECK(pc.sizes() == g.sizes() && pc.scalar_type() == g.scalar_type(), "bias_grad: pre mismatch");
  }
  at::hip::HIPGuardMasqueradingAsCUDA guard(dy.device());
  if (pc.defined()) dp = at::empty_like(g);
  else dp = at::empty({0}, g.options());
  const int R = madnn_bias_grad_rows(M, (int)N, pc.defined() ? 1 : 0);
  at::Tensor partial = at::empty({R, N}, g.options().dtype(at::kFloat));
  at::Tensor db = at::empty({N}, g.options().dtype(bias_dtype));
  check(madnn_bias_grad(g.data_ptr(), pc.defined() ? pc.data_ptr() : nullptr, pc.defined() ? dp.data_ptr() : nullptr,
                        M, (int)N, dt_code(g), partial.data_ptr<float>(), db.data_ptr(), dt_code(db), (int)gelu_kind,
                        cur_stream(g)),
        "bias_grad");
  return {db, dp};
}

at::Tensor gelu_fwd(const at::Tensor& x, int64_t kind) {
  TORCH_CHECK(kind == 1 || kind == 2, "gelu_fwd: kind 1 (tanh) or 2 (erf)");
  check_dev(x, "x");
  at::Tensor xc = x.contiguous();
  TORCH_CHECK(xc.numel() % 8 == 0, "gelu_fwd: numel must be a multiple of 8");
  at::hip::HIPGuardMasqueradingAsCUDA guard(x.device());
  at::Tensor y = at::empty_like(xc);
  if (xc.numel())
    check(madnn_gelu_fwd(xc.data_ptr(), y.data_ptr(), xc.numel(), dt_code(xc), (int)kind, cur_stream(xc)), "gelu_fwd");
  return y;
}

static void check_aligned16(const at::Tensor& t, const char* op, const char* name) {
  TORCH_CHECK(reinterpret_cast<uintptr_t>(t.data_ptr()) % 16 == 0, op, ": ", name, " must be 16-byte aligned");
}

at::Tensor rope_qkv_impl(const at::Tensor& qkv, at::Tensor out, const at::Tensor& cos, const at::Tensor& sin,
                         int64_t rot_heads, bool inverse) {
  check_dev(qkv, "qkv");
  TORCH_CHECK(qkv.scalar_type() == at::kBFloat16 && qkv.dim() == 4 && qkv.is_contiguous(),
              "rope_qkv_: qkv must be a contiguous bf16 [B, S, heads, D]");
  const int64_t S = qkv.size(1), NH = qkv.size(2), D = qkv.size(3);
  TORCH_CHECK(D % 16 == 0 && rot_heads >= 0 && rot_heads <= NH, "rope_qkv_: D % 16 and rot_heads <= heads");
  for (const at::Tensor* t : {&cos, &sin}) {
    TORCH_CHECK(t->device() == qkv.device() && t->scalar_type() == at::kFloat && t->dim() == 2 && t->is_contiguous() &&
                    t->size(0) >= S && t->size(1) == D,
                "rope_qkv_: cos / sin must be contiguous fp32 [>= S, D] on the device");
  }
  for (const at::Tensor* t : {&qkv, const_cast<const at::Tensor*>(&out), &cos, &sin}) check_aligned16(*t, "rope_qkv", "qkv / out / cos / sin");
  at::hip::HIPGuardMasqueradingAsCUDA guard(qkv.device());
  check(madnn_rope_qkv(qkv.data_ptr(), out.data_ptr(), cos.data_ptr<float>(), sin.data_ptr<float>(), qkv.size(0) * S,
                       (int)S, (int)NH, (int)rot_heads, (int)D, inverse ? 1 : 0, cur_stream(qkv)),
        "rope_qkv");
  return out;
}

at::Tensor rope_qkv_(at::Tensor qkv, const at::Tensor& cos, const at::Tensor& sin, int64_t rot_heads, bool inverse) {
  return rope_qkv_impl(qkv, qkv, cos, sin, rot_heads, inverse);
}

at::Tensor rope_qkv(const at::Tensor& qkv, const at::Tensor& cos, const at::Tensor& sin, int64_t rot_heads,
                    bool inverse) {
  check_dev(qkv, "qkv");
  return rope_qkv_impl(qkv, at::empty_like(qkv), cos, sin, rot_heads, inverse);
}

at::Tensor swiglu_fwd(const at::Tensor& gu) {
  check_dev(gu, "gu");
  TORCH_CHECK(gu.scalar_type() == at::kBFloat16 && gu.is_contiguous() && gu.size(-1) % 16 == 0,
              "swiglu: gu must be contiguous bf16 with a last dim that is a multiple of 16");
  const int64_t I = gu.size(-1) / 2, M = gu.numel() / (2 * I);
  auto shape = gu.sizes().vec();
  shape.back() = I;
  check_aligned16(gu, "swiglu", "gu");
  at::hip::HIPGuardMasqueradingAsCUDA guard(gu.device());
  at::Tensor h = at::empty(shape, gu.options());
  check(madnn_swiglu_fwd(gu.data_ptr(), h.data_ptr(), M, (int)I, cur_stream(gu)), "swiglu_fwd");
  return h;
}

at::Tensor swiglu_bwd(const at::Tensor& dh, const at::Tensor& gu) {
  check_dev(gu, "gu");
  TORCH_CHECK(gu.scalar_type() == at::kBFloat16 && gu.is_contiguous() && gu.size(-1) % 16 == 0, "swiglu_bwd: gu");
  const int64_t I = gu.size(-1) / 2, M = gu.numel() / (2 * I);
  at::Tensor d = dh.to(at::kBFloat16).contiguous();
  TORCH_CHECK(d.numel() == M * I, "swiglu_bwd: dh must have gu's rows and I columns");
  check_aligned16(gu, "swiglu_bwd", "gu");
  check_aligned16(d, "swiglu_bwd", "dh");
  at::hip::HIPGuardMasqueradingAsCUDA guard(gu.device());
  at::Tensor dgu = at::empty_like(gu);
  check(madnn_swiglu_bwd(d.data_ptr(), gu.data_ptr(), dgu.data_ptr(), M, (int)I, cur_stream(gu)), "swiglu_bwd");
  return dgu;
}

void attn_check(const at::Tensor& t, const char* name, int64_t D) {
  check_dev(t, name);
  TORCH_CHECK(t.scalar_type() == at::kBFloat16, "attention: ", name, " must be bf16");
  TORCH_CHECK(t.dim() == 4 && t.size(3) == D && t.stride(3) == 1, "attention: ", name, " must be [B, S, heads, D]");
  for (int i = 0; i < 3; ++i) TORCH_CHECK(t.stride(i) % 8 == 0, "attention: ", name, " strides must be multiples of 8");
  TORCH_CHECK(reinterpret_cast<uintptr_t>(t.data_ptr()) % 16 == 0, "attention: ", name, " must be 16-byte aligned");
}

MadnnAttnArgs attn_args(const at::Tensor& q, const at::Tensor& k, const at::Tensor& v, double scale) {
  const int64_t D = q.size(3);
  TORCH_CHECK(madnn_attn_supported((int)D), "attention: head dim must be 64 or 128");
  attn_check(q, "q", D);
  attn_check(k, "k", D);
  attn_check(v, "v", D);
  TORCH_CHECK(k.sizes() == v.sizes() && k.size(0) == q.size(0) && k.size(1) == q.size(1), "attention: k/v shape");
  TORCH_CHECK(q.size(2) % k.size(2) == 0, "attention: query heads must be a multiple of kv heads");
  TORCH_CHECK(q.size(1) < (1ll << 30) && q.size(0) * q.size(2) < (1ll << 30), "attention: problem too large");
  MadnnAttnArgs a{};
  a.q = reinterpret_cast<const uint16_t*>(q.data_ptr());
  a.k = reinterpret_cast<const uint16_t*>(k.data_ptr());
  a.v = reinterpret_cast<const uint16_t*>(v.data_ptr());
  a.q_sb = q.stride(0); a.q_ss = q.stride(1); a.q_sh = q.stride(2);
  a.k_sb = k.stride(0); a.k_ss = k.stride(1); a.k_sh = k.stride(2);
  a.v_sb = v.stride(0); a.v_ss = v.stride(1); a.v_sh = v.stride(2);
  a.B = (int)q.size(0); a.S = (int)q.size(1); a.H = (int)q.size(2); a.Hkv = (int)k.size(2);
  a.scale = (float)scale;
  a.scale_log2 = (float)(scale * 1.4426950408889634);
// ... 20 lines not shown
  const int64_t D = q.size(3);
  TORCH_CHECK(o.is_contiguous() && o.sizes() == q.sizes(), "attn_bwd: o must be contiguous [B, S, H, D]");
  at::Tensor doc = dout.contiguous();
  TORCH_CHECK(doc.sizes() == o.sizes() && doc.scalar_type() == at::kBFloat16, "attn_bwd: grad shape/dtype");
  attn_check(dq, "dq", D);
  attn_check(dk, "dk", D);
  attn_check(dv, "dv", D);
  TORCH_CHECK(dq.sizes() == q.sizes() && dk.sizes() == k.sizes() && dv.sizes() == v.sizes(), "attn_bwd: grad shapes");
  TORCH_CHECK(lse.is_contiguous() && lse.numel() == q.size(0) * q.size(1) * q.size(2), "attn_bwd: lse");
  at::hip::HIPGuardMasqueradingAsCUDA guard(q.device());
  at::Tensor delta = at::empty_like(lse);
  a.o = reinterpret_cast<uint16_t*>(o.data_ptr());
  a.lse = lse.data_ptr<float>();
  a.dout = reinterpret_cast<const uint16_t*>(doc.data_ptr());
  a.delta = delta.data_ptr<float>();
  a.o_sb = o.stride(0); a.o_ss = o.stride(1); a.o_sh = o.stride(2);
  a.dq = reinterpret_cast<uint16_t*>(dq.data_ptr());
  a.dk = reinterpret_cast<uint16_t*>(dk.data_ptr());
  a.dv = reinterpret_cast<uint16_t*>(dv.data_ptr());
  a.dq_sb = dq.stride(0); a.dq_ss = dq.stride(1); a.dq_sh = dq.stride(2);
  a.dk_sb = dk.stride(0); a.dk_ss = dk.stride(1); a.dk_sh = dk.stride(2);
  a.dv_sb = dv.stride(0); a.dv_ss = dv.stride(1); a.dv_sh = dv.stride(2);
  const bool cs = colsum.has_value() && colsum->defined();
  at::Tensor cpart;
  int64_t R = 0, C = 0;
  if (cs) {
    C = (q.size(2) + 2 * k.size(2)) * D;
    TORCH_CHECK((colsum->scalar_type() == at::kFloat || colsum->scalar_type() == at::kBFloat16) &&
                    colsum->is_contiguous() && colsum->numel() == C,
                "attn_bwd: colsum must be a contiguous fp32 / bf16 [(H + 2 Hkv) * D]");
    R = madnn_attn_colsum_rows(a.B, a.S);
    cpart = at::empty({R, C}, q.options().dtype(at::kFloat));
    a.cpart = cpart.data_ptr<float>();
  }
  check(madnn_attn_bwd(&a, (int)D, causal ? 1 : 0, cur_stream(q)), "attn_bwd");
  if (cs)
    check(madnn_attn_colsum_finalize(a.cpart, R, C, colsum->data_ptr(), colsum->scalar_type() == at::kBFloat16 ? 1 : 0,
                                     cur_stream(q)),
          "attn_colsum");
}

void hwq_wait(const at::Tensor& flag, int64_t expect, int64_t timeout_us, at::Tensor out) {
  check_dev(flag, "flag");
  check_dev(out, "out");
  TORCH_CHECK(flag.scalar_type() == at::kInt && out.scalar_type() == at::kInt && out.numel() >= 2 &&
                  out.is_contiguous() && timeout_us > 0 && timeout_us <= 2000000,
              "hwq_wait: int32 flag, int32 out[>=2], 0 < timeout_us <= 2 s");
  at::hip::HIPGuardMasqueradingAsCUDA guard(flag.device());
  check(madnn_hwq_wait(flag.data_ptr<int>(), (int)expect, timeout_us, out.data_ptr<int>(), cur_stream(flag)),
        "hwq_wait");
}

void hwq_set(at::Tensor flag, int64_t val) {
  check_dev(flag, "flag");
  TORCH_CHECK(flag.scalar_type() == at::kInt, "hwq_set: int32 flag");
  at::hip::HIPGuardMasqueradingAsCUDA guard(flag.device());
  check(madnn_hwq_set(flag.data_ptr<int>(), (int)val, cur_stream(flag)), "hwq_set");
}

void hwq_batch(const at::Tensor& kinds, const at::Tensor& msgs, at::Tensor a, at::Tensor b, int64_t epoch,
               int64_t timeout_us, at::Tensor ok, const at::Tensor& ok_index) {
  for (const at::Tensor* t : {&kinds, &msgs, static_cast<const at::Tensor*>(&a), static_cast<const at::Tensor*>(&b),
                              static_cast<const at::Tensor*>(&ok), &ok_index}) {
    check_dev(*t, "hwq_batch operand");
    TORCH_CHECK(t->scalar_type() == at::kInt && t->is_contiguous(), "hwq_batch: contiguous int32 operands");
  }
  const int64_t n = kinds.numel();
  TORCH_CHECK(msgs.numel() == n && ok_index.numel() == n && timeout_us > 0 && timeout_us <= 2000000,
              "hwq_batch: kinds / msgs / ok_index of one length, 0 < timeout_us <= 2 s");
  at::hip::HIPGuardMasqueradingAsCUDA guard(a.device());
  check(madnn_hwq_batch(kinds.data_ptr<int>(), msgs.data_ptr<int>(), (int)n, a.data_ptr<int>(), b.data_ptr<int>(),
                        (int)epoch, timeout_us, ok.data_ptr<int>(), ok_index.data_ptr<int>(), cur_stream(a)),
        "hwq_batch");
}

void hwq_spin(const at::Tensor& like, int64_t spin_us) {
  check_dev(like, "like");
  TORCH_CHECK(spin_us >= 0 && spin_us <= 100000, "hwq_spin: 0 <= spin_us <= 100 ms");
  at::hip::HIPGuardMasqueradingAsCUDA guard(like.device());
  check(madnn_hwq_spin(spin_us, cur_stream(like)), "hwq_spin");
}

}

TORCH_LIBRARY(madnn, m) {
  m.def("hwq_batch(Tensor kinds, Tensor msgs, Tensor(a!) a, Tensor(b!) b, int epoch, int timeout_us, Tensor(c!) ok, "
        "Tensor ok_index) -> ()");
  m.def("hwq_spin(Tensor like, int spin_us) -> ()");
  m.def("hwq_wait(Tensor flag, int expect, int timeout_us, Tensor(a!) out) -> ()");
  m.def("hwq_set(Tensor(a!) flag, int val) -> ()");
  m.def(
      "bn_fwd(Tensor x, Tensor? res, Tensor? w, Tensor? b, Tensor(a!)? run_mean, Tensor(b!)? run_var, "
      "Tensor(c!)? nbt, bool training, float momentum, float eps, bool relu, Tensor? partial=None) -> (Tensor, Tensor, "
      "Tensor, Tensor, Tensor, Tensor)");
  m.def("xent_fwd(Tensor logits, Tensor targets, bool shift, int V, int ignore_index) -> (Tensor, Tensor)");
  m.def(
      "xent_bwd(Tensor logits, Tensor targets, Tensor lse, bool shift, int V, int ignore_index, Tensor gscale) -> "
      "Tensor");
  m.def(
      "xent_fused(Tensor logits, Tensor targets, bool shift, int V, int ignore_index, Tensor gscale) -> "
      "(Tensor, Tensor)");
  m.def("xent_rescale(Tensor(a!) grad, Tensor g) -> ()");
  m.def(
      "bn_bwd(Tensor dy, Tensor x, Tensor? mask, bool has_res, Tensor? w, Tensor save_mean, Tensor save_invstd, "
      "Tensor scale, Tensor shift, bool relu, bool need_wgrad, bool write_dres=True) -> (Tensor, Tensor, Tensor, Tensor)");
  m.def(
      "bn_fwd_dual(Tensor x, Tensor r, Tensor? w, Tensor? b, Tensor(a!)? run_mean, Tensor(b!)? run_var, "
      "Tensor(c!)? nbt, float momentum, float eps, Tensor? partial, Tensor? w_r, Tensor? b_r, "
      "Tensor(d!)? run_mean_r, Tensor(e!)? run_var_r, Tensor(f!)? nbt_r, float momentum_r, float eps_r, "
      "Tensor? partial_r) -> Tensor[]");
  m.def(
      "bn_bwd_dual(Tensor dy, Tensor x, Tensor r, Tensor mask, Tensor? w, Tensor save_mean, Tensor save_invstd, "
      "Tensor? w_r, Tensor save_mean_r, Tensor save_invstd_r) -> Tensor[]");
  m.def("attn_fwd(Tensor q, Tensor k, Tensor v, bool causal, float scale) -> (Tensor, Tensor)");
  m.def(
      "attn_bwd(Tensor dout, Tensor q, Tensor k, Tensor v, Tensor o, Tensor lse, Tensor(a!) dq, Tensor(b!) dk, "
      "Tensor(c!) dv, bool causal, float scale, Tensor(d!)? colsum=None) -> ()");
  m.def("conv1x1_fwd(Tensor x, Tensor w, bool stats) -> (Tensor, Tensor)");
  m.def("conv1x1_dgrad(Tensor dy, Tensor w, Tensor? res=None, Tensor? resmask=None) -> Tensor");
  m.def("conv1x1_dgrad_bnb(Tensor dy, Tensor w, Tensor bny, Tensor scale, Tensor shift) -> (Tensor, Tensor)");
  m.def(
      "conv3x3_fwd_bnb(Tensor x, Tensor w, Tensor bny, Tensor scale, Tensor shift) -> (Tensor, Tensor)");
  m.def(
      "bn_bwd_ext(Tensor dy, Tensor x, Tensor? w, Tensor save_mean, Tensor save_invstd, Tensor scale, Tensor shift, "
      "Tensor partial, bool relu) -> (Tensor, Tensor, Tensor)");
  m.def("conv1x1_wgrad(Tensor dy, Tensor x, bool out_bf16=False) -> Tensor");
  m.def(
      "bn_bwd_coef(Tensor dy, Tensor x, Tensor mask, Tensor? w, Tensor save_mean, Tensor save_invstd, Tensor scale, "
      "Tensor shift) -> (Tensor, Tensor, Tensor)");
  m.def(
      "bn_bwd_dual_coef(Tensor dy, Tensor x, Tensor r, Tensor mask, Tensor? w, Tensor save_mean, Tensor save_invstd, "
      "Tensor? w_r, Tensor save_mean_r, Tensor save_invstd_r) -> Tensor[]");
  m.def("bn3_conv3_bwd_supported(int c, int c4) -> bool", &bn3_conv3_bwd_supported);
  m.def(
      "bn3_conv3_bwd(Tensor dout, Tensor y3, Tensor mask, Tensor coef, Tensor w3, Tensor a2, Tensor? y2, "
      "Tensor? scale2, Tensor? shift2, bool dw_bf16) -> (Tensor, Tensor, Tensor)");
  m.def(
      "bn_coef(Tensor x, Tensor? w, Tensor? b, Tensor(a!)? run_mean, Tensor(b!)? run_var, Tensor(c!)? nbt, "
      "float momentum, float eps, Tensor? partial=None) -> Tensor[]");
  m.def("stem_fwd(Tensor x, Tensor wp, bool stats) -> (Tensor, Tensor)");
  m.def("linear_fwd(Tensor x, Tensor w, Tensor? bias, Tensor? res, int act, bool save_aux) -> (Tensor, Tensor)");
  m.def("linear_dgrad(Tensor dy, Tensor w, Tensor? res, bool accumulate) -> Tensor");
  m.def("linear_wgrad(Tensor dy, Tensor x, Tensor? out, bool accumulate, int splits) -> Tensor");
  m.def("linear_wgrad4(Tensor dy, Tensor x, Tensor? out, bool accumulate, int splits) -> Tensor");
  m.def("linear_wgrad4h(Tensor dy, Tensor x, Tensor? out, bool accumulate, int splits) -> Tensor");
  m.def("wgrad_splits(int M, int N, int K) -> int", &wgrad_splits);
  m.def("gemmp_supported(int I, int J, int K, bool has_bias) -> bool", &gemmp_supported);
  m.def("linear_fwd_p(Tensor x, Tensor w, Tensor? bias, int act) -> (Tensor, Tensor)");
  m.def("linear_dgrad_p(Tensor dy, Tensor w, Tensor? pre, ScalarType bias_dtype, int gelu_kind=1) -> (Tensor, Tensor)");
  m.def("conv3x3_fwd(Tensor x, Tensor w, bool stats) -> (Tensor, Tensor)");
  m.def("conv3x3_fwd_s2(Tensor x, Tensor w, bool stats) -> (Tensor, Tensor)");
  m.def("conv3x3_wgrad(Tensor dy, Tensor x, bool out_bf16) -> Tensor");
  m.def("stem_wgrad(Tensor dy, Tensor x) -> Tensor");
  m.def("bias_grad(Tensor dy, Tensor? pre, ScalarType bias_dtype, int gelu_kind=1) -> (Tensor, Tensor)");
  m.def("gelu_fwd(Tensor x, int kind=1) -> Tensor");
  m.def("rope_qkv_(Tensor(a!) qkv, Tensor cos, Tensor sin, int rot_heads, bool inverse) -> Tensor(a!)");
  m.def("rope_qkv(Tensor qkv, Tensor cos, Tensor sin, int rot_heads, bool inverse) -> Tensor");
  m.def("swiglu_fwd(Tensor gu) -> Tensor");
  m.def("swiglu_bwd(Tensor dh, Tensor gu) -> Tensor");
  m.def("maxpool_fwd(Tensor x, int k, int s, int p, bool need_arg) -> (Tensor, Tensor)");
  m.def("pool_bn_fwd(Tensor y, Tensor scale, Tensor shift, int p) -> (Tensor, Tensor)");
  m.def(
      "pool_bn_bwd(Tensor dp, Tensor arg, Tensor y, Tensor? w, Tensor mean, Tensor invstd, Tensor scale, Tensor shift, "
      "int p) -> (Tensor, Tensor, Tensor)");
  m.def("maxpool_bwd(Tensor dy, Tensor arg, int H, int W, int k, int s, int p) -> Tensor");
  m.def("bucket_pack(Tensor[] srcs, Tensor(a!) flat, int[] offsets, float scale) -> ()");
  m.def("bucket_unpack(Tensor(a!)[] dsts, Tensor flat, int[] offsets, float scale) -> ()");
  m.def("flat_scale_cast(Tensor src, Tensor(a!) dst, float scale) -> ()");
  m.def(
      "sgd_step(Tensor(a!) master, Tensor grad, Tensor(b!)? mom, Tensor(c!)? model, float lr, float momentum, "
      "float dampening, float weight_decay, bool nesterov, bool first_step, float grad_scale, Tensor? dscale) -> ()");
  m.def(
      "adam_step(Tensor(a!) master, Tensor grad, Tensor(b!) m1, Tensor(c!) m2, Tensor(d!)? model, float lr, "
      "float beta1, float beta2, float eps, float weight_decay, bool adamw, int step, float grad_scale, "
      "Tensor? dscale) -> ()");
  m.def("grad_norm(Tensor[] flats, float max_norm, float scale) -> Tensor");
  m.def("norm_fwd(Tensor x, Tensor? res, Tensor w, Tensor? b, float eps, bool rms) -> (Tensor, Tensor, Tensor, Tensor)");
  m.def(
      "norm_bwd(Tensor dy, Tensor x, Tensor w, Tensor mean, Tensor rstd, Tensor? dres, bool rms, bool has_bias, "
      "bool colsum=False, bool colsum_bf16=False) -> (Tensor, Tensor, Tensor, Tensor)");
}

TORCH_LIBRARY_IMPL(madnn, CUDA, m) {
  m.impl("bucket_pack", bucket_pack);
  m.impl("bucket_unpack", bucket_unpack);
  m.impl("flat_scale_cast", flat_scale_cast);
  m.impl("sgd_step", sgd_step);
  m.impl("adam_step", adam_step);
  m.impl("grad_norm", grad_norm);
  m.impl("norm_fwd", norm_fwd);
  m.impl("norm_bwd", norm_bwd);
  m.impl("bn_fwd", bn_fwd);
  m.impl("bn_bwd", bn_bwd);
  m.impl("bn_fwd_dual", bn_fwd_dual);
  m.impl("bn_coef", bn_coef);
  m.impl("conv3x3_fwd_bnb", conv3x3_fwd_bnb);
  m.impl("conv1x1_dgrad_bnb", conv1x1_dgrad_bnb);
  m.impl("bn_bwd_ext", bn_bwd_ext);
  m.impl("bn_bwd_dual", bn_bwd_dual);
  m.impl("xent_fwd", xent_fwd);
  m.impl("xent_bwd", xent_bwd);
  m.impl("xent_fused", xent_fused);
  m.impl("xent_rescale", xent_rescale);
  m.impl("maxpool_fwd", maxpool_fwd);
  m.impl("pool_bn_fwd", pool_bn_fwd);
  m.impl("pool_bn_bwd", pool_bn_bwd);
  m.impl("bias_grad", bias_grad);
  m.impl("gelu_fwd", gelu_fwd);
  m.impl("rope_qkv_", rope_qkv_);
  m.impl("rope_qkv", rope_qkv);
  m.impl("swiglu_fwd", swiglu_fwd);
  m.impl("swiglu_bwd", swiglu_bwd);
  m.impl("attn_fwd", attn_fwd);
  m.impl("attn_bwd", attn_bwd);
  m.impl("maxpool_bwd", maxpool_bwd);
  m.impl("conv1x1_fwd", conv1x1_fwd);
  m.impl("conv1x1_dgrad", conv1x1_dgrad);
  m.impl("conv1x1_wgrad", conv1x1_wgrad);
  m.impl("bn_bwd_coef", bn_bwd_coef);
  m.impl("bn_bwd_dual_coef", bn_bwd_dual_coef);
  m.impl("bn3_conv3_bwd", bn3_conv3_bwd);
  m.impl("stem_fwd", stem_fwd);
  m.impl("stem_wgrad", stem_wgrad);
  m.impl("linear_fwd", linear_fwd);
  m.impl("linear_dgrad", linear_dgrad);
  m.impl("linear_wgrad", linear_wgrad);
  m.impl("linear_wgrad4", linear_wgrad4);
  m.impl("linear_wgrad4h", linear_wgrad4h);
  m.impl("linear_fwd_p", linear_fwd_p);
  m.impl("linear_dgrad_p", linear_dgrad_p);
  m.impl("conv3x3_fwd", conv3x3_fwd);
  m.impl("conv3x3_fwd_s2", conv3x3_fwd_s2);
  m.impl("conv3x3_wgrad", conv3x3_wgrad);
  m.impl("hwq_wait", hwq_wait);
  m.impl("hwq_set", hwq_set);
  m.impl("hwq_batch", hwq_batch);
  m.impl("hwq_spin", hwq_spin);
}
```

madnn/ops/csrc/pool.hip:

```cpp
#include "common.h"

namespace madnn {

template <int XDT>
__global__ __launch_bounds__(256) void maxpool_fwd_kernel(const void* __restrict__ x, void* __restrict__ y,
                                                          uint64_t* __restrict__ arg, int N, int H, int W, int C,
                                                          int Ho, int Wo, int k, int s, int p) {
  const unsigned CG = (unsigned)C >> 3;
  const unsigned total = (unsigned)N * Ho * Wo * CG;
  for (unsigned idx = blockIdx.x * blockDim.x + threadIdx.x; idx < total; idx += gridDim.x * blockDim.x) {
    const unsigned cg = idx % CG;
    const unsigned pix = idx / CG;
    const int ow = (int)(pix % (unsigned)Wo);
    const unsigned t = pix / (unsigned)Wo;
    const int oh = (int)(t % (unsigned)Ho);
    const int n = (int)(t / (unsigned)Ho);
    const int h0 = oh * s - p, w0 = ow * s - p;
    const int kh0 = h0 < 0 ? -h0 : 0, kw0 = w0 < 0 ? -w0 : 0;
    const int kh1 = min(k, H - h0), kw1 = min(k, W - w0);
    float best[8];
    unsigned char a[8];
    const unsigned char first = (unsigned char)(kh0 * k + kw0);
#pragma unroll
    for (int j = 0; j < 8; ++j) {
      best[j] = -__builtin_inff();
      a[j] = first;
    }
    for (int kh = kh0; kh < kh1; ++kh) {
      const unsigned rowbase = ((unsigned)(n * H + h0 + kh) * W) * C + cg * 8;
      for (int kw = kw0; kw < kw1; ++kw) {
        float v[8];
        load8<XDT>(x, rowbase + (unsigned)(w0 + kw) * C, v);
        const unsigned char pos = (unsigned char)(kh * k + kw);
#pragma unroll
        for (int j = 0; j < 8; ++j) {
          if (v[j] > best[j] || __builtin_isnan(v[j])) {
            best[j] = v[j];
            a[j] = pos;
          }
        }
      }
    }
    store8<XDT>(y, (int64_t)pix * C + cg * 8, best);
    if (arg) {
      uint64_t packed = 0;
#pragma unroll
      for (int j = 0; j < 8; ++j) packed |= (uint64_t)a[j] << (8 * j);
      arg[idx] = packed;
    }
  }
}

template <int XDT>
__global__ __launch_bounds__(256) void maxpool_bwd_kernel(const void* __restrict__ dy,
                                                          const uint64_t* __restrict__ arg, void* __restrict__ dx,
                                                          int N, int H, int W, int C, int Ho, int Wo, int k, int s,
                                                          int p) {
  const unsigned CG = (unsigned)C >> 3;
  const unsigned total = (unsigned)N * H * W * CG;
  for (unsigned idx = blockIdx.x * blockDim.x + threadIdx.x; idx < total; idx += gridDim.x * blockDim.x) {
    const unsigned cg = idx % CG;
    const unsigned pix = idx / CG;
    const int w = (int)(pix % (unsigned)W);
    const unsigned t = pix / (unsigned)W;
    const int h = (int)(t % (unsigned)H);
    const int n = (int)(t / (unsigned)H);
    const int nh = h + p - (k - 1), nw = w + p - (k - 1);
    const int oh_lo = nh <= 0 ? 0 : (nh + s - 1) / s;
    const int ow_lo = nw <= 0 ? 0 : (nw + s - 1) / s;
    const int oh_hi = min(Ho - 1, (h + p) / s);
    const int ow_hi = min(Wo - 1, (w + p) / s);
    float acc[8];
#pragma unroll
    for (int j = 0; j < 8; ++j) acc[j] = 0.f;
    for (int oh = oh_lo; oh <= oh_hi; ++oh) {
      for (int ow = ow_lo; ow <= ow_hi; ++ow) {
        const unsigned oidx = ((unsigned)(n * Ho + oh) * Wo + ow) * CG + cg;
        const uint64_t packed = arg[oidx];
        const unsigned pos = (unsigned)((h - (oh * s - p)) * k + (w - (ow * s - p)));
        float g[8];
        load8<XDT>(dy, (int64_t)oidx * 8, g);
#pragma unroll
        for (int j = 0; j < 8; ++j) acc[j] += (((packed >> (8 * j)) & 0xffu) == pos) ? g[j] : 0.f;
      }
    }
    store8<XDT>(dx, (int64_t)idx * 8, acc);
  }
}

__device__ __forceinline__ unsigned xcd_block_id(int swz) {
  if (!swz) return blockIdx.x;
  return (blockIdx.x % kNumXCD) * (gridDim.x / kNumXCD) + blockIdx.x / kNumXCD;
}

template <int XDT, bool BNRELU = false>
__global__ __launch_bounds__(256) void maxpool_k3s2_fwd_kernel(const void* __restrict__ x, void* __restrict__ y,
                                                               uint64_t* __restrict__ arg, int N, int H, int W,
                                                               int C, int Ho, int Wo, int p, int swz,
                                                               const float* __restrict__ sc = nullptr,
                                                               const float* __restrict__ sh = nullptr) {
  const unsigned CG = (unsigned)C >> 3;
  const unsigned total = (unsigned)N * Ho * Wo * CG;
  for (unsigned idx = xcd_block_id(swz) * blockDim.x + threadIdx.x; idx < total; idx += gridDim.x * blockDim.x) {
    const unsigned cg = idx % CG;
    const unsigned pix = idx / CG;
    const int ow = (int)(pix % (unsigned)Wo);
    const unsigned t = pix / (unsigned)Wo;
    const int oh = (int)(t % (unsigned)Ho);
    const int n = (int)(t / (unsigned)Ho);
    const int h0 = oh * 2 - p, w0 = ow * 2 - p;
    float v[9][8];
    bool ok[9];
    float bs[8], bh[8];
    if constexpr (BNRELU) {
      load8<kF32>(sc, cg * 8, bs);
      load8<kF32>(sh, cg * 8, bh);
    }
#pragma unroll
    for (int kh = 0; kh < 3; ++kh) {
#pragma unroll
      for (int kw = 0; kw < 3; ++kw) {
        const int h = h0 + kh, w = w0 + kw;
        const int q = kh * 3 + kw;
        ok[q] = (unsigned)h < (unsigned)H && (unsigned)w < (unsigned)W;
        if (ok[q]) {
          load8<XDT>(x, ((unsigned)(n * H + h) * W + (unsigned)w) * C + cg * 8, v[q]);
        }
      }
    }
    if constexpr (BNRELU) {
#pragma unroll
      for (int q = 0; q < 9; ++q) {
        if (!ok[q]) continue;
#pragma unroll
        for (int j = 0; j < 8; ++j) {
          const float z = v[q][j] * bs[j] + bh[j];
          v[q][j] = z > 0.f ? z : 0.f;
        }
      }
    }
    float best[8];
    unsigned char a[8];
    unsigned char first = 0;
#pragma unroll
    for (int q = 8; q >= 0; --q)
      if (ok[q]) first = (unsigned char)q;
#pragma unroll
    for (int j = 0; j < 8; ++j) {
      best[j] = -__builtin_inff();
      a[j] = first;
    }
#pragma unroll
    for (int q = 0; q < 9; ++q) {
      if (!ok[q]) continue;
#pragma unroll
      for (int j = 0; j < 8; ++j) {
        if (v[q][j] > best[j] || __builtin_isnan(v[q][j])) {
          best[j] = v[q][j];
          a[j] = (unsigned char)q;
        }
      }
    }
    store8<XDT>(y, (int64_t)pix * C + cg * 8, best);
    if (arg) {
      uint64_t packed = 0;
#pragma unroll
      for (int j = 0; j < 8; ++j) packed |= (uint64_t)a[j] << (8 * j);
      arg[idx] = packed;
    }
  }
}

template <int XDT>
__global__ __launch_bounds__(256) void maxpool_k3s2_bwd_kernel(const void* __restrict__ dy,
                                                               const uint64_t* __restrict__ arg,
                                                               void* __restrict__ dx, int N, int H, int W, int C,
                                                               int Ho, int Wo, int p, int swz) {
  const unsigned CG = (unsigned)C >> 3;
  const unsigned total = (unsigned)N * H * W * CG;
  for (unsigned idx = xcd_block_id(swz) * blockDim.x + threadIdx.x; idx < total; idx += gridDim.x * blockDim.x) {
    const unsigned cg = idx % CG;
    const unsigned pix = idx / CG;
    const int w = (int)(pix % (unsigned)W);
    const unsigned t = pix / (unsigned)W;
    const int h = (int)(t % (unsigned)H);
    const int n = (int)(t / (unsigned)H);
    const int oh1 = (h + p) >> 1, ow1 = (w + p) >> 1;
    uint64_t pk[4];
    float g[4][8];
    unsigned pos[4];
    bool ok[4];
#pragma unroll
    for (int i = 0; i < 2; ++i) {
#pragma unroll
      for (int j = 0; j < 2; ++j) {
        const int oh = oh1 - 1 + i, ow = ow1 - 1 + j;
        const int dh = h - (oh * 2 - p), dw = w - (ow * 2 - p);
        const int q = i * 2 + j;
        ok[q] = oh >= 0 && oh < Ho && ow >= 0 && ow < Wo && dh <= 2 && dw <= 2;
        pos[q] = (unsigned)(dh * 3 + dw);
        if (ok[q]) {
          const unsigned oidx = ((unsigned)(n * Ho + oh) * Wo + ow) * CG + cg;
          pk[q] = arg[oidx];
          load8<XDT>(dy, (int64_t)oidx * 8, g[q]);
        }
      }
    }
    float acc[8];
#pragma unroll
    for (int j = 0; j < 8; ++j) acc[j] = 0.f;
#pragma unroll
    for (int q = 0; q < 4; ++q) {
      if (!ok[q]) continue;
#pragma unroll
      for (int j = 0; j < 8; ++j) acc[j] += (((pk[q] >> (8 * j)) & 0xffu) == pos[q]) ? g[q][j] : 0.f;
    }
    store8<XDT>(dx, (int64_t)idx * 8, acc);
  }
}

template <int PHASE>
__global__ __launch_bounds__(256) void pool_bn_bwd_kernel(const void* __restrict__ dp, const uint64_t* __restrict__ arg,
                                                          const void* __restrict__ y, const float* __restrict__ sc,
                                                          const float* __restrict__ sh, const float* __restrict__ ca,
                                                          const float* __restrict__ cb, const float* __restrict__ cc,
                                                          void* __restrict__ dy, float* __restrict__ partial, int N,
                                                          int H, int W, int C, int Ho, int Wo, int p) {
  __shared__ float slab[256][17];
  const unsigned CG = (unsigned)C >> 3;
  const unsigned total = (unsigned)N * H * W * CG;
  const unsigned cg = threadIdx.x % CG;
  float bs[8], bh[8], s0[8], s1[8], k0[8], k1[8], k2[8];
  load8<kF32>(sc, cg * 8, bs);
  load8<kF32>(sh, cg * 8, bh);
  if constexpr (PHASE == 1) {
    load8<kF32>(ca, cg * 8, k0);
    load8<kF32>(cb, cg * 8, k1);
    load8<kF32>(cc, cg * 8, k2);
  }
#pragma unroll
  for (int j = 0; j < 8; ++j) s0[j] = s1[j] = 0.f;
  for (unsigned idx = blockIdx.x * blockDim.x + threadIdx.x; idx < total; idx += gridDim.x * blockDim.x) {
    const unsigned pix = idx / CG;
    const int w = (int)(pix % (unsigned)W);
    const unsigned t = pix / (unsigned)W;
    const int h = (int)(t % (unsigned)H);
    const int n = (int)(t / (unsigned)H);
    const int oh1 = (h + p) >> 1, ow1 = (w + p) >> 1;
    uint64_t pk[4];
    float g[4][8];
    unsigned pos[4];
    bool ok[4];
#pragma unroll
    for (int i = 0; i < 2; ++i) {
#pragma unroll
      for (int j = 0; j < 2; ++j) {
        const int oh = oh1 - 1 + i, ow = ow1 - 1 + j;
        const int dh = h - (oh * 2 - p), dw = w - (ow * 2 - p);
        const int q = i * 2 + j;
        ok[q] = oh >= 0 && oh < Ho && ow >= 0 && ow < Wo && dh <= 2 && dw <= 2;
        pos[q] = (unsigned)(dh * 3 + dw);
        if (ok[q]) {
          const unsigned oidx = ((unsigned)(n * Ho + oh) * Wo + ow) * CG + cg;
          pk[q] = arg[oidx];
          load8<kBF16>(dp, (int64_t)oidx * 8, g[q]);
        }
      }
    }
    float yv[8];
    load8<kBF16>(y, (int64_t)idx * 8, yv);
    float acc[8];
#pragma unroll
    for (int j = 0; j < 8; ++j) acc[j] = 0.f;
#pragma unroll
    for (int q = 0; q < 4; ++q) {
      if (!ok[q]) continue;
#pragma unroll
      for (int j = 0; j < 8; ++j) acc[j] += (((pk[q] >> (8 * j)) & 0xffu) == pos[q]) ? g[q][j] : 0.f;
    }
#pragma unroll
    for (int j = 0; j < 8; ++j) {
      const float z = yv[j] * bs[j] + bh[j];
      acc[j] = z > 0.f ? acc[j] : 0.f;
    }
    if constexpr (PHASE == 0) {
#pragma unroll
      for (int j = 0; j < 8; ++j) {
        s0[j] += acc[j];
        s1[j] += acc[j] * yv[j];
      }
    } else {
      float o[8];
#pragma unroll
      for (int j = 0; j < 8; ++j) o[j] = k0[j] * acc[j] + k1[j] * yv[j] + k2[j];
      store8<kBF16>(dy, (int64_t)idx * 8, o);
    }
  }
  if constexpr (PHASE == 0) {
#pragma unroll
    for (int j = 0; j < 8; ++j) {
      slab[threadIdx.x][j] = s0[j];
      slab[threadIdx.x][8 + j] = s1[j];
    }
    __syncthreads();
    for (int c = threadIdx.x; c < 2 * C; c += blockDim.x) {
      const int which = c / C, ch = c % C, g8 = ch >> 3, e = ch & 7;
      float a = 0.f;
      for (int r = g8; r < 256; r += (int)CG) a += slab[r][which * 8 + e];
      partial[(int64_t)blockIdx.x * 2 * C + c] = a;
    }
  }
}

}

using namespace madnn;

static int g_pool_k3s2 = 1;

extern "C" {

int madnn_maxpool_set_k3s2(int on) {
  const int old = g_pool_k3s2;
  if (on >= 0) g_pool_k3s2 = on;
  return old;
}

int madnn_maxpool_supported(int64_t numel, int C, int k) { return numel < (1ll << 31) && C % 8 == 0 && k * k <= 255; }

hipError_t madnn_maxpool_fwd(const void* x, void* y, void* arg, int N, int H, int W, int C, int Ho, int Wo, int k,
                             int s, int p, int xdt, hipStream_t stream) {
  const int64_t work = (int64_t)N * Ho * Wo * (C / 8);
  const int grid = stream_grid(work, 256, 16 * kNumCU);
  if (k == 3 && s == 2 && p <= 2 && g_pool_k3s2) {
    const int g8 = (grid + kNumXCD - 1) / kNumXCD * kNumXCD;
    MADNN_DISPATCH_DT(xdt, XDT, {
      hipLaunchKernelGGL((maxpool_k3s2_fwd_kernel<XDT>), dim3(g_pool_k3s2 == 2 ? g8 : grid), dim3(256), 0, stream, x, y,
                         static_cast<uint64_t*>(arg), N, H, W, C, Ho, Wo, p,
                         (int)(g_pool_k3s2 == 2));
    });
    return hipGetLastError();
  }
  MADNN_DISPATCH_DT(xdt, XDT, {
    hipLaunchKernelGGL((maxpool_fwd_kernel<XDT>), dim3(grid), dim3(256), 0, stream, x, y,
                       static_cast<uint64_t*>(arg), N, H, W, C, Ho, Wo, k, s, p);
  });
  return hipGetLastError();
}

hipError_t madnn_maxpool_bwd(const void* dy, const void* arg, void* dx, int N, int H, int W, int C, int Ho, int Wo,
                             int k, int s, int p, int xdt, hipStream_t stream) {
  const int64_t work = (int64_t)N * H * W * (C / 8);
  const int grid = stream_grid(work, 256, 16 * kNumCU);
  if (k == 3 && s == 2 && p <= 2 && g_pool_k3s2) {
    const int g8 = (grid + kNumXCD - 1) / kNumXCD * kNumXCD;
    MADNN_DISPATCH_DT(xdt, XDT, {
      hipLaunchKernelGGL((maxpool_k3s2_bwd_kernel<XDT>), dim3(g_pool_k3s2 == 2 ? g8 : grid), dim3(256), 0, stream, dy,
                         static_cast<const uint64_t*>(arg), dx, N, H, W, C, Ho, Wo, p,
                         (int)(g_pool_k3s2 == 2));
    });
    return hipGetLastError();
  }
  MADNN_DISPATCH_DT(xdt, XDT, {
    hipLaunchKernelGGL((maxpool_bwd_kernel<XDT>), dim3(grid), dim3(256), 0, stream, dy,
                       static_cast<const uint64_t*>(arg), dx, N, H, W, C, Ho, Wo, k, s, p);
  });
  return hipGetLastError();
}


static int g_pool_bn_wg[3] = {16, 8, 16};

int madnn_pool_bn_tune(int key, int value) {
  if (key < 0 || key > 2) return -1;
  const int old = g_pool_bn_wg[key];
  if (value > 0) g_pool_bn_wg[key] = value;
  return old;
}

int madnn_pool_bn_supported(int64_t numel, int C) {
  return numel < (1ll << 31) && C % 8 == 0 && C <= 2048 && 256 % (C / 8) == 0;
}

hipError_t madnn_pool_bn_fwd(const void* x, const float* scale, const float* shift, void* y, void* arg, int N, int H,
                             int W, int C, int Ho, int Wo, int p, hipStream_t stream) {
  if (!madnn_pool_bn_supported((int64_t)N * H * W * C, C) || p > 2) return hipErrorInvalidValue;
  const int64_t work = (int64_t)N * Ho * Wo * (C / 8);
  const int grid = stream_grid(work, 256, g_pool_bn_wg[0] * kNumCU);
  hipLaunchKernelGGL((maxpool_k3s2_fwd_kernel<kBF16, true>), dim3(grid), dim3(256), 0, stream, x, y,
                     static_cast<uint64_t*>(arg), N, H, W, C, Ho, Wo, p, 0, scale, shift);
  return hipGetLastError();
}

hipError_t madnn_bn_bwd_finalize(const float* partial, int G, int C, int pstride, int qoff, int64_t M, const float* w,
                                 const float* mean, const float* invstd, float* dw, float* db, float* ca, float* cb,
                                 float* cc, hipStream_t stream);

int madnn_pool_bn_bwd_rows(int64_t pixels, int C) {
  const int64_t work = pixels * (C / 8);
  return stream_grid(work, 256, g_pool_bn_wg[1] * kNumCU);
}

hipError_t madnn_pool_bn_bwd(const void* dp, const void* arg, const void* y, const float* w, const float* mean,
                             const float* invstd, const float* scale, const float* shift, void* dy, float* dw,
                             float* db, float* coef, float* workspace, int N, int H, int W, int C, int Ho, int Wo,
                             int p, hipStream_t stream) {
  if (!madnn_pool_bn_supported((int64_t)N * H * W * C, C) || p > 2) return hipErrorInvalidValue;
  const int64_t pixels = (int64_t)N * H * W;
  const int G = madnn_pool_bn_bwd_rows(pixels, C);
  const uint64_t* a = static_cast<const uint64_t*>(arg);
  hipLaunchKernelGGL((pool_bn_bwd_kernel<0>), dim3(G), dim3(256), 0, stream, dp, a, y, scale, shift, nullptr, nullptr,
                     nullptr, nullptr, workspace, N, H, W, C, Ho, Wo, p);
  MADNN_HIP_CHECK(hipGetLastError());
  MADNN_HIP_CHECK(madnn_bn_bwd_finalize(workspace, G, C, 2 * C, C, pixels, w, mean, invstd, dw, db, coef, coef + C,
                                        coef + 2 * C, stream));
  const int grid = stream_grid(pixels * (C / 8), 256, g_pool_bn_wg[2] * kNumCU);
  hipLaunchKernelGGL((pool_bn_bwd_kernel<1>), dim3(grid), dim3(256), 0, stream, dp, a, y, scale, shift, coef, coef + C,
                     coef + 2 * C, dy, nullptr, N, H, W, C, Ho, Wo, p);
  return hipGetLastError();
}

}
```

madnn/ops/csrc/stem.hip:

```cpp
#include "mfma.h"

namespace madnn {
namespace stem {

using namespace mf;

constexpr int kThreads = 256;
constexpr int kCo = 64;
constexpr int kKh = 7;
constexpr int kKp = 224;
constexpr int kSteps = kKp / 16;
constexpr int kMaxWo = 128;

struct StemArgs {
  const uint16_t* x;
  const uint16_t* w;
  uint16_t* y;
  float* stats;
  int N, H, W, Ho, Wo;
  int rows;
};

__device__ __forceinline__ int img_elem(int kh, int px, int c, int WP) { return (kh * WP + px) * 4 + c; }

// ... 4 lines not shown
  const int IMG = kKh * WP * 4;
  uint16_t* img0 = smem;
  uint16_t* img1 = smem + IMG;
  char* otile = reinterpret_cast<char*>(smem + 2 * IMG);
  const int tid = threadIdx.x, wave = tid >> 6, lane = tid & 63, l32 = lane & 31, hh = lane >> 5;
  const int row_elems = a.W * 3;
  const int chunks = (row_elems + 7) / 8;
  const int PER = (kKh * chunks + kThreads - 1) / kThreads;

  for (int i = tid; i < IMG; i += kThreads) {
    img0[i] = 0;
    img1[i] = 0;
  }

  const int nb = wave & 1, pb0 = 64 * (wave >> 1);
  bf16x8 wf[kSteps];
#pragma unroll
  for (int s = 0; s < kSteps; ++s)
    wf[s] = *reinterpret_cast<const bf16x8*>(a.w + (32 * nb + l32) * kKp + 16 * s + 8 * hh);

  float ssum[8], ssq[8];
  if constexpr (STATS) {
#pragma unroll
    for (int e = 0; e < 8; ++e) ssum[e] = ssq[e] = 0.f;
  }

  u32x4 stg[4];
  auto load = [&](int row) {
    const int n = row / a.Ho, oh = row % a.Ho;
#pragma unroll
    for (int i = 0; i < 4; ++i) {
      const int c = tid + kThreads * i;
      stg[i] = u32x4{0u, 0u, 0u, 0u};
      if (i < PER && c < kKh * chunks) {
        const int kh = c / chunks, ch = c % chunks;
        const int ih = 2 * oh - 3 + kh;
        if (ih >= 0 && ih < a.H) {
          stg[i] = *reinterpret_cast<const u32x4*>(a.x + ((int64_t)n * a.H + ih) * row_elems + ch * 8);
        }
      }
    }
  };
  auto store = [&](uint16_t* img) {
#pragma unroll
    for (int i = 0; i < 4; ++i) {
      const int c = tid + kThreads * i;
      if (i < PER && c < kKh * chunks) {
        const int kh = c / chunks, ch = c % chunks;
#pragma unroll
        for (int k = 0; k < 8; ++k) {
          const int e = ch * 8 + k;
          const unsigned v = (stg[i][k >> 1] >> (16 * (k & 1))) & 0xffffu;
          img[img_elem(kh, e / 3 + 3, e % 3, WP)] = (uint16_t)v;
        }
      }
    }
  };

  int row = blockIdx.x;
  if (row >= a.rows) return;
  __syncthreads();
  load(row);
  store(img0);
  __syncthreads();
  int cur = 0;
  for (;;) {
    const int nrow = row + gridDim.x;
    const bool more = nrow < a.rows;
    if (more) load(nrow);
    const uint16_t* img = cur ? img1 : img0;
    f32x16 acc[2] = {zero16(), zero16()};
    if (pb0 < a.Wo) {
#pragma unroll
      for (int kh = 0; kh < kKh; ++kh)
#pragma unroll
        for (int s2 = 0; s2 < 2; ++s2) {
#pragma unroll
          for (int q = 0; q < 2; ++q) {
            const int pix = min(pb0 + 32 * q + l32, a.Wo - 1);
            const int px = 2 * pix + 4 * s2 + 2 * hh;
            const bf16x8 bx = *reinterpret_cast<const bf16x8*>(img + img_elem(kh, px, 0, WP));
            acc[q] = mfma(wf[2 * kh + s2], bx, acc[q]);
          }
        }
    }
#pragma unroll
    for (int q = 0; q < 2; ++q) {
      const int pix = pb0 + 32 * q + l32;
#pragma unroll
      for (int g = 0; g < 4; ++g) {
        const int co = 32 * nb + 8 * g + 4 * hh;
        const unsigned lo = (unsigned)f32_to_bf16(acc[q][4 * g]) | ((unsigned)f32_to_bf16(acc[q][4 * g + 1]) << 16);
        const unsigned hi = (unsigned)f32_to_bf16(acc[q][4 * g + 2]) | ((unsigned)f32_to_bf16(acc[q][4 * g + 3]) << 16);
        *reinterpret_cast<u32x2*>(otile + pix * 128 + 16 * ((co >> 3) ^ ((pix >> 1) & 7)) + 8 * ((co >> 2) & 1)) =
            u32x2{lo, hi};
      }
    }
    __syncthreads();
    {
      uint16_t* yrow = a.y + (int64_t)row * a.Wo * kCo;
      const int c = tid & 7;
      for (int r = tid >> 3; r < a.Wo; r += kThreads / 8) {
        const u32x4 v = *reinterpret_cast<const u32x4*>(otile + r * 128 + 16 * (c ^ ((r >> 1) & 7)));
        *reinterpret_cast<u32x4*>(yrow + r * kCo + 8 * c) = v;
        if constexpr (STATS) {
#pragma unroll
          for (int e = 0; e < 4; ++e) {
            const float x0 = bf16_to_f32((unsigned short)(v[e] & 0xffffu));
            const float x1 = bf16_to_f32((unsigned short)(v[e] >> 16));
            ssum[2 * e] += x0;
            ssq[2 * e] += x0 * x0;
            ssum[2 * e + 1] += x1;
            ssq[2 * e + 1] += x1 * x1;
          }
        }
      }
    }
    if (!more) break;
    store(cur ? img0 : img1);
    __syncthreads();
    cur ^= 1;
    row = nrow;
  }

  if constexpr (STATS) {
    __syncthreads();
    float* red = reinterpret_cast<float*>(otile);
    const int c = tid & 7, rg = tid >> 3;
#pragma unroll
    for (int e = 0; e < 8; ++e) {
      red[(rg * 2) * kCo + 8 * c + e] = ssum[e];
      red[(rg * 2 + 1) * kCo + 8 * c + e] = ssq[e];
    }
    __syncthreads();
    if (tid < 2 * kCo) {
      const int which = tid / kCo, co = tid % kCo;
      float v = 0.f;
      for (int g = 0; g < kThreads / 8; ++g) v += red[(g * 2 + which) * kCo + co];
      a.stats[((int64_t)blockIdx.x * 2 + which) * kCo + co] = v;
    }
  }
}

inline int stem_grid(int rows) { return rows < 2 * kNumCU ? rows : 2 * kNumCU; }

constexpr int kWMaxTiles = 4;

struct StemWArgs {
  const uint16_t* x;
  const uint16_t* dy;
  float* ws;
  int N, H, W, Ho, Wo;
  int rows, per;
};

__device__ __forceinline__ bf16x8 lds_patch(const uint16_t* img_row, int ow0, int lane) {
  const int g = lane >> 4, i = lane & 15;
  const int kw = 4 * (g & 1) + (i & 3);
  const int ow = ow0 + 8 * (g >> 1) + (i >> 2);
  typedef __attribute__((address_space(3))) s16x4 lds_s16x4;
  const uint16_t* p = img_row + (2 * ow + kw) * 4;
  const s16x4 lo = __builtin_amdgcn_ds_read_tr16_b64_v4i16((lds_s16x4*)p);
  const s16x4 hi = __builtin_amdgcn_ds_read_tr16_b64_v4i16((lds_s16x4*)(p + 8 * 4));
  const s16x8 r = {lo[0], lo[1], lo[2], lo[3], hi[0], hi[1], hi[2], hi[3]};
  return __builtin_bit_cast(bf16x8, r);
}

__global__ __launch_bounds__(kThreads, 2) void stem_wgrad_kernel(const StemWArgs a) {
  extern __shared__ __attribute__((aligned(16))) uint16_t smem[];
  const int WOP = (a.Wo + 15) & ~15;
  const int ROW = (2 * WOP + 6) * 4;
  uint16_t* ring = smem;
  uint16_t* dyt = smem + 9 * ROW;
  const int tid = threadIdx.x, wave = tid >> 6, lane = tid & 63, hh = lane >> 5, l32 = lane & 31;
  const int row_elems = a.W * 3, chunks = row_elems / 8;
  const int dchunks = a.Wo * 8;

  const int r0 = blockIdx.x * a.per;
  const int r1 = min(r0 + a.per, a.rows);
  if (r0 >= r1) return;
  for (int i = tid; i < 9 * ROW + WOP * kCo; i += kThreads) smem[i] = 0;

  const int b = wave & 1, kh0 = wave >> 1;
  f32x16 acc[kWMaxTiles];
#pragma unroll
  for (int q = 0; q < kWMaxTiles; ++q) acc[q] = zero16();

  u32x4 istg[4], dstg[4];
  int s_oh = 0, s_klo = 0;
  auto load = [&](int r) {
    const int n = r / a.Ho, oh = r % a.Ho;
    const bool fresh = (r == r0) || (oh == 0);
    s_oh = oh;
    s_klo = fresh ? 0 : 5;
    const int total = (kKh - s_klo) * chunks;
#pragma unroll
    for (int i = 0; i < 4; ++i) {
      const int c = tid + kThreads * i;
      istg[i] = u32x4{0u, 0u, 0u, 0u};
      if (c < total) {
        const int ih = 2 * oh - 3 + s_klo + c / chunks;
        if (ih >= 0 && ih < a.H)
          istg[i] = *reinterpret_cast<const u32x4*>(a.x + ((int64_t)n * a.H + ih) * row_elems + (c % chunks) * 8);
      }
      const int d = tid + kThreads * i;
      if (d < dchunks) dstg[i] = *reinterpret_cast<const u32x4*>(a.dy + ((int64_t)r * a.Wo) * kCo + d * 8);
    }
  };
  auto store = [&]() {
    const int total = (kKh - s_klo) * chunks;
#pragma unroll
    for (int i = 0; i < 4; ++i) {
      const int c = tid + kThreads * i;
      if (c < total) {
        const int ih = 2 * s_oh - 3 + s_klo + c / chunks, ch = c % chunks;
        if (ih >= 0 && ih < a.H) {
          uint16_t* img = ring + (ih & 7) * ROW;
#pragma unroll
          for (int k = 0; k < 8; ++k) {
            const int e = ch * 8 + k;
            img[(e / 3 + 3) * 4 + e % 3] = (uint16_t)((istg[i][k >> 1] >> (16 * (k & 1))) & 0xffffu);
          }
        }
      }
      const int d = tid + kThreads * i;
      if (d < dchunks)
        *reinterpret_cast<u32x4*>(reinterpret_cast<char*>(dyt) + swz<64>(d >> 3, d & 7)) = dstg[i];
    }
  };

  __syncthreads();
  load(r0);
  store();
  __syncthreads();
  for (int r = r0;;) {
    const int oh = r % a.Ho;
    const bool more = r + 1 < r1;
    if (more) load(r + 1);
    const uint16_t* rows_kh[kWMaxTiles];
#pragma unroll
    for (int q = 0; q < kWMaxTiles; ++q) {
      const int ih = 2 * oh - 3 + kh0 + 2 * q;
      rows_kh[q] = ring + ((ih >= 0 && ih < a.H) ? (ih & 7) : 8) * ROW;
    }
    for (int t = 0; t < WOP; t += 16) {
      const bf16x8 af = lds_col<64>(dyt, t, 32 * b, lane);
#pragma unroll
      for (int q = 0; q < kWMaxTiles; ++q)
        if (kh0 + 2 * q < kKh) acc[q] = mfma(af, lds_patch(rows_kh[q], t, lane), acc[q]);
    }
    if (!more) break;
    __syncthreads();
    store();
    __syncthreads();
    ++r;
  }

  const int kw = l32 >> 2, c = l32 & 3;
  if (kw < 7 && c < 3) {
    float* out = a.ws + (int64_t)blockIdx.x * kCo * 147;
#pragma unroll
    for (int q = 0; q < kWMaxTiles; ++q) {
      const int kh = kh0 + 2 * q;
      if (kh < kKh) {
#pragma unroll
        for (int e = 0; e < 16; ++e) {
          const int co = 32 * b + acc_row(e, hh);
          out[co * 147 + c * 49 + kh * 7 + kw] = acc[q][e];
        }
      }
    }
  }
}

__global__ __launch_bounds__(256) void stem_wgrad_reduce(const float* __restrict__ ws, float* __restrict__ dw, int parts) {
  __shared__ float red[8][32];
  const int col = threadIdx.x & 31, grp = threadIdx.x >> 5;
  const int i = blockIdx.x * 32 + col;
  const int64_t stride = (int64_t)kCo * 147;
  float s[8] = {0.f, 0.f, 0.f, 0.f, 0.f, 0.f, 0.f, 0.f};
  if (i < kCo * 147) {
    int g = grp;
    for (; g + 56 < parts; g += 64) {
#pragma unroll
      for (int u = 0; u < 8; ++u) s[u] += ws[(int64_t)(g + 8 * u) * stride + i];
    }
    for (; g < parts; g += 8) s[0] += ws[(int64_t)g * stride + i];
  }
  red[grp][col] = ((s[0] + s[1]) + (s[2] + s[3])) + ((s[4] + s[5]) + (s[6] + s[7]));
  __syncthreads();
  if (grp == 0 && i < kCo * 147) {
    float t = 0.f;
#pragma unroll
    for (int k = 0; k < 8; ++k) t += red[k][col];
    dw[i] = t;
  }
}

inline int wgrad_grid(int rows) { return rows < 2 * kNumCU ? rows : 2 * kNumCU; }

}
}

using namespace madnn::stem;

extern "C" {

int madnn_stem_supported(int H, int W) {
  const int Wo = (W + 6 - 7) / 2 + 1;
  return (H >= 7 && W >= 8 && W % 8 == 0 && Wo <= kMaxWo && kKh * (W * 3 / 8) <= 4 * kThreads) ? 1 : 0;
}

int madnn_stem_stat_rows(int N, int H, int W) {
  const int Ho = (H + 6 - 7) / 2 + 1;
  return stem_grid(N * Ho);
}

hipError_t madnn_stem_fwd(const void* x, const void* wp, void* y, float* stats, int N, int H, int W, hipStream_t s) {
  if (!madnn_stem_supported(H, W)) return hipErrorInvalidValue;
  StemArgs a{};
  a.x = static_cast<const uint16_t*>(x);
  a.w = static_cast<const uint16_t*>(wp);
  a.y = static_cast<uint16_t*>(y);
  a.stats = stats;
  a.N = N;
  a.H = H;
  a.W = W;
  a.Ho = (H + 6 - 7) / 2 + 1;
  a.Wo = (W + 6 - 7) / 2 + 1;
  a.rows = N * a.Ho;
  if (a.rows <= 0) return hipSuccess;
  const int WP = 2 * a.Wo + 6;
  const size_t lds = (size_t)2 * kKh * WP * 4 * sizeof(uint16_t) + (size_t)kMaxWo * kCo * sizeof(uint16_t);
  const int grid = stem_grid(a.rows);
  if (stats) {
    hipLaunchKernelGGL(stem_fwd_kernel<true>, dim3(grid), dim3(kThreads), lds, s, a);
  } else {
    hipLaunchKernelGGL(stem_fwd_kernel<false>, dim3(grid), dim3(kThreads), lds, s, a);
  }
  return hipGetLastError();
}

int64_t madnn_stem_wgrad_ws(int N, int H, int W) {
  const int Ho = (H + 6 - 7) / 2 + 1;
  return (int64_t)wgrad_grid(N * Ho) * kCo * 147;
}

hipError_t madnn_stem_wgrad(const void* x, const void* dy, float* ws, float* dw, int N, int H, int W,
                            hipStream_t s) {
  if (!madnn_stem_supported(H, W)) return hipErrorInvalidValue;
  StemWArgs a{};
  a.x = static_cast<const uint16_t*>(x);
  a.dy = static_cast<const uint16_t*>(dy);
  a.ws = ws;
  a.N = N;
  a.H = H;
  a.W = W;
  a.Ho = (H + 6 - 7) / 2 + 1;
  a.Wo = (W + 6 - 7) / 2 + 1;
  a.rows = N * a.Ho;
  if (a.rows <= 0) return hipMemsetAsync(dw, 0, sizeof(float) * kCo * 147, s);
  a.per = (a.rows + wgrad_grid(a.rows) - 1) / wgrad_grid(a.rows);
  const int grid = (a.rows + a.per - 1) / a.per;
  const int WOP = (a.Wo + 15) & ~15;
  const size_t lds = (size_t)(9 * (2 * WOP + 6) * 4 + WOP * kCo) * sizeof(uint16_t);
  hipLaunchKernelGGL(stem_wgrad_kernel, dim3(grid), dim3(kThreads), lds, s, a);
  MADNN_HIP_CHECK(hipGetLastError());
  hipLaunchKernelGGL(stem_wgrad_reduce, dim3((kCo * 147 + 31) / 32), dim3(256), 0, s, ws, dw, grid);
  return hipGetLastError();
}

}
```

Before: 13920.

## Fuse stem BN/ReLU/maxpool backward into the stem weight-gradient kernel

Adds a fused stem path for ResNet. The forward runs conv, BN coefficients and pool in sequence and also saves a gathered y-at-argmax map. The backward computes BN coefficients from the pooled gradient alone, then rebuilds the full-resolution conv-output gradient on the fly inside the stem wgrad kernel from the pooled gradient, argmax bytes and saved y. This avoids materialising and rereading the large full-resolution dy tensor and drops a separate pool/BN backward pass. The cost is extra LDS and ALU work in the wgrad kernel. The path applies only when the input does not require grad, which holds for the stem.

```diff
diff --git a/madnn/models/resnet.py b/madnn/models/resnet.py
--- a/madnn/models/resnet.py
+++ b/madnn/models/resnet.py
@@ -13,7 +13,8 @@
 from ..ops import (batch_norm_add_bn_relu, bn2_conv3_bn3_add_bn_relu, bn2_conv3_bn3_add_bn_relu_supported,
                    bn2_conv3_bn3_add_relu, bn2_conv3_bn3_supported, bn_relu_conv1x1,
                    bn_relu_conv1x1_epi_supported, bn_relu_conv3x3, bn_relu_conv3x3_supported, bn_relu_maxpool,
-                   bn_relu_maxpool_supported, conv1x1_route, defer_res_mask)
+                   bn_relu_maxpool_supported, conv1x1_route, defer_res_mask, stem_bn_relu_maxpool,
+                   stem_bn_relu_maxpool_supported)
 
 _FORK_DS = os.environ.get("MADNN_FORK_DOWNSAMPLE", "1") != "0"
 _DUAL_BN = os.environ.get("MADNN_DUAL_BN", "1") != "0"
@@ -185,7 +186,14 @@
         layers += [block(self.inplanes, planes) for _ in range(1, blocks)]
         return nn.Sequential(*layers)
 
+    def _stem_fused(self, x) -> bool:
+        return (isinstance(x, torch.Tensor) and isinstance(self.conv1, FusedConv2d) and isinstance(self.bn1, BN)
+                and isinstance(self.maxpool, FusedMaxPool2d) and self.conv1.stem_ok(x)
+                and stem_bn_relu_maxpool_supported(x, self.conv1.weight, self.bn1, self.maxpool))
+
     def stem(self, x):
+        if self._stem_fused(x):
+            return stem_bn_relu_maxpool(x, self.conv1.weight, self.bn1, self.maxpool)
         y, st = self.conv1(x, stats=True)
         if isinstance(self.bn1, BN) and isinstance(self.maxpool, FusedMaxPool2d) \
                 and bn_relu_maxpool_supported(y, self.bn1, self.maxpool):
diff --git a/madnn/nn/conv.py b/madnn/nn/conv.py
--- a/madnn/nn/conv.py
+++ b/madnn/nn/conv.py
@@ -31,6 +31,9 @@
                 and self.dilation == (1, 1) and self.groups == 1 and self.bias is None
                 and ops.stem_supported(x, self.weight))
 
+    def stem_ok(self, x: torch.Tensor) -> bool:
+        return self._k10(x)
+
     def forward(self, x: torch.Tensor, stats: bool = False, fork: bool = False):
         if self._k9(x):
             return ops.conv1x1(x, self.weight, stats=stats, fork=fork)
diff --git a/madnn/ops/__init__.py b/madnn/ops/__init__.py
--- a/madnn/ops/__init__.py
+++ b/madnn/ops/__init__.py
@@ -890,12 +890,16 @@
         return dy, dw, db, None, None, None
 
 
-def bn_relu_maxpool_supported(y: torch.Tensor, bn, pool) -> bool:
-    return (_POOL_BN and isinstance(y, torch.Tensor) and y.device.type == "cuda" and y.dtype == torch.bfloat16 and y.dim() == 4
-            and y.is_contiguous(memory_format=torch.channels_last) and _bn_trainable(bn)
+def _bn_relu_maxpool_modules_ok(bn, pool) -> bool:
+    return (_POOL_BN and _bn_trainable(bn)
             and _pair(pool.kernel_size) == (3, 3) and _pair(pool.stride) == (2, 2)
             and _pair(pool.padding) in ((1, 1), (0, 0)) and _pair(pool.dilation) == (1, 1)
-            and not pool.ceil_mode and not pool.return_indices
+            and not pool.ceil_mode and not pool.return_indices)
+
+
+def bn_relu_maxpool_supported(y: torch.Tensor, bn, pool) -> bool:
+    return (isinstance(y, torch.Tensor) and y.device.type == "cuda" and y.dtype == torch.bfloat16 and y.dim() == 4
+            and y.is_contiguous(memory_format=torch.channels_last) and _bn_relu_maxpool_modules_ok(bn, pool)
             and y.size(1) % 8 == 0 and 256 % (y.size(1) // 8) == 0 and y.numel() < 2 ** 31)
 
 
@@ -1100,6 +1104,49 @@
     _need_native("stem_conv")
     y, part = _StemFn.apply(x, w, stats)
     return (y, part) if stats else y
+
+
+class _StemBNReluMaxPoolFn(torch.autograd.Function):
+
+    @staticmethod
+    def forward(ctx, x, w, bn_w, bn_b, bn, p):
+        y, part = torch.ops.madnn.stem_fwd(x, _stem_pack(w), True)
+        mean, invstd, scale, shift = torch.ops.madnn.bn_coef(y, bn_w, bn_b, bn.running_mean, bn.running_var,
+                                                             bn.num_batches_tracked, float(bn.momentum),
+                                                             float(bn.eps), part)
+        out, arg, yarg = torch.ops.madnn.pool_bn_fwd_yarg(y, scale, shift, int(p))
+        ctx.save_for_backward(x, w, y, arg, yarg, bn_w, mean, invstd, scale, shift)
+        ctx.p = int(p)
+        return out
+
+    @staticmethod
+    def backward(ctx, dp):
+        x, w, y, arg, yarg, bn_w, mean, invstd, scale, shift = ctx.saved_tensors
+        dp = _like(dp, yarg)
+        coef, dbw, dbb = torch.ops.madnn.pool_bn_bwd_coef(dp, yarg, bn_w, mean, invstd, scale, shift,
+                                                          y.numel() // y.size(1))
+        dw = None
+        if ctx.needs_input_grad[1]:
+            dw = _like(torch.ops.madnn.stem_wgrad_bnp(x, y, dp, arg, scale, shift, coef, ctx.p).to(w.dtype), w)
+        need = ctx.needs_input_grad[2] or ctx.needs_input_grad[3]
+        return None, dw, dbw if need else None, dbb if need else None, None, None
+
+
+_STEM_BWD_FUSED = os.environ.get("MADNN_STEM_BWD_FUSED", "1") != "0"
+
+
+def stem_bn_relu_maxpool_supported(x: torch.Tensor, w: torch.Tensor, bn, pool) -> bool:
+    if not (_STEM_BWD_FUSED and isinstance(x, torch.Tensor) and stem_supported(x, w) and w.size(0) == 64
+            and not x.requires_grad and torch.is_grad_enabled() and _bn_relu_maxpool_modules_ok(bn, pool)
+            and bn.weight.numel() == 64 and native_available()):
+        return False
+    ho, wo, p = (x.size(2) - 1) // 2 + 1, (x.size(3) - 1) // 2 + 1, _pair(pool.padding)[0]
+    return ho + 2 * p >= 3 and wo + 2 * p >= 3 and x.size(0) * 64 * ho * wo < 2 ** 31
+
+
+def stem_bn_relu_maxpool(x: torch.Tensor, w: torch.Tensor, bn, pool) -> torch.Tensor:
+    _need_native("stem_bn_relu_maxpool")
+    return _StemBNReluMaxPoolFn.apply(x, w, bn.weight, bn.bias, bn, _pair(pool.padding)[0])
 
 
 def hidden_supported(h: int) -> bool:
@@ -1616,7 +1663,7 @@
     "max_pool2d", "max_pool_supported", "conv1x1", "conv1x1_route", "batch_norm_add_bn_relu",
     "batch_norm_dual_supported", "bn_relu_conv1x1", "bn_relu_maxpool",
     "bn_relu_maxpool_supported", "bn_relu_conv3x3", "bn_relu_conv3x3_supported",
-    "bn_relu_conv1x1_epi_supported", "bn2_conv3_bn3_add_relu", "bn2_conv3_bn3_supported", "bn2_conv3_bn3_add_bn_relu", "bn2_conv3_bn3_add_bn_relu_supported", "conv1x1_supported", "stem_conv", "stem_supported", "native_available", "load_kernels", "kernels_path", "hidden_supported", "reference",
+    "bn_relu_conv1x1_epi_supported", "bn2_conv3_bn3_add_relu", "bn2_conv3_bn3_supported", "bn2_conv3_bn3_add_bn_relu", "bn2_conv3_bn3_add_bn_relu_supported", "conv1x1_supported", "stem_conv", "stem_supported", "stem_bn_relu_maxpool", "stem_bn_relu_maxpool_supported", "native_available", "load_kernels", "kernels_path", "hidden_supported", "reference",
     "linear", "linear_tee", "gelu_mlp", "bias_grad", "gelu_tanh", "grad_sink", "wgrad_into", "tuned_wgrad", "dgrad",
     "dgrad_dgelu", "load_tuning_table", "export_choices", "sync_choices", "tuning_timings", "tuning_measurements",
 ]
diff --git a/madnn/ops/csrc/binding.cpp b/madnn/ops/csrc/binding.cpp
--- a/madnn/ops/csrc/binding.cpp
+++ b/madnn/ops/csrc/binding.cpp
@@ -45,8 +45,11 @@
 hipError_t madnn_maxpool_fwd(const void*, void*, void*, int, int, int, int, int, int, int, int, int, int, hipStream_t);
 int madnn_pool_bn_supported(int64_t, int);
 int madnn_pool_bn_bwd_rows(int64_t, int);
-hipError_t madnn_pool_bn_fwd(const void*, const float*, const float*, void*, void*, int, int, int, int, int, int, int,
-                             hipStream_t);
+int madnn_pool_bn_bwd_pooled_rows(int64_t, int);
+hipError_t madnn_pool_bn_fwd(const void*, const float*, const float*, void*, void*, void*, int, int, int, int, int, int,
+                             int, hipStream_t);
+hipError_t madnn_pool_bn_bwd_pooled(const void*, const void*, const float*, const float*, const float*, const float*,
+                                    const float*, float*, float*, float*, float*, int64_t, int64_t, int, hipStream_t);
 hipError_t madnn_pool_bn_bwd(const void*, const void*, const void*, const float*, const float*, const float*,
                              const float*, const float*, void*, float*, float*, float*, float*, int, int, int, int, int,
                              int, int, hipStream_t);
@@ -96,6 +99,9 @@
 hipError_t madnn_stem_fwd(const void*, const void*, void*, float*, int, int, int, hipStream_t);
 int64_t madnn_stem_wgrad_ws(int, int, int);
 hipError_t madnn_stem_wgrad(const void*, const void*, float*, float*, int, int, int, hipStream_t);
+hipError_t madnn_stem_wgrad_bnp(const void*, const void*, const void*, const void*, const float*, const float*,
+                                const float*, const float*, const float*, float*, float*, int, int, int, int,
+                                hipStream_t);
 int madnn_gemm_supported(int64_t, int64_t, int64_t, int64_t, int64_t);
 int madnn_conv3x3_supported(int, int, int, int);
 int madnn_conv3x3_stat_rows(int64_t);
@@ -1056,6 +1062,36 @@
   return dw;
 }
 
+at::Tensor stem_wgrad_bnp(const at::Tensor& x, const at::Tensor& y, const at::Tensor& dp, const at::Tensor& arg,
+                          const at::Tensor& scale, const at::Tensor& shift, const at::Tensor& coef, int64_t p) {
+  stem_check_x(x);
+  check_dev(y, "y");
+  check_dev(dp, "dp");
+  check_dev(arg, "arg");
+  const int N = (int)x.size(0), H = (int)x.size(2), W = (int)x.size(3);
+  const int64_t Ho = (H - 1) / 2 + 1, Wo = (W - 1) / 2 + 1;
+  TORCH_CHECK(p >= 0 && p <= 1 && Ho + 2 * p >= 3 && Wo + 2 * p >= 3, "stem_wgrad_bnp: unsupported pool");
+  const int64_t Hp = (Ho + 2 * p - 3) / 2 + 1, Wp = (Wo + 2 * p - 3) / 2 + 1;
+  TORCH_CHECK(y.scalar_type() == at::kBFloat16 && y.dim() == 4 && y.size(0) == N && y.size(1) == 64 &&
+                  y.size(2) == Ho && y.size(3) == Wo && y.is_contiguous(at::MemoryFormat::ChannelsLast),
+              "stem_wgrad_bnp: y must be channels_last bf16 [N, 64, Ho, Wo]");
+  TORCH_CHECK(dp.scalar_type() == at::kBFloat16 && dp.dim() == 4 && dp.size(0) == N && dp.size(1) == 64 &&
+                  dp.size(2) == Hp && dp.size(3) == Wp && dp.is_contiguous(at::MemoryFormat::ChannelsLast),
+              "stem_wgrad_bnp: dp must be channels_last bf16 [N, 64, Hp, Wp]");
+  TORCH_CHECK(arg.scalar_type() == at::kByte && arg.is_contiguous() && arg.numel() == dp.numel(),
+              "stem_wgrad_bnp: argmax map mismatch");
+  const float* sc = vec_ptr(scale, 64, "stem_wgrad_bnp", "scale");
+  const float* sh = vec_ptr(shift, 64, "stem_wgrad_bnp", "shift");
+  const float* cf = vec_ptr(coef, 3 * 64, "stem_wgrad_bnp", "coef");
+  at::hip::HIPGuardMasqueradingAsCUDA guard(x.device());
+  at::Tensor ws = at::empty({madnn_stem_wgrad_ws(N, H, W)}, x.options().dtype(at::kFloat));
+  at::Tensor dw = at::empty({64, 3, 7, 7}, x.options().dtype(at::kFloat));
+  check(madnn_stem_wgrad_bnp(x.data_ptr(), y.data_ptr(), dp.data_ptr(), arg.data_ptr(), sc, sh, cf, cf + 64, cf + 128,
+                             ws.data_ptr<float>(), dw.data_ptr<float>(), N, H, W, (int)p, cur_stream(x)),
+        "stem_wgrad_bnp");
+  return dw;
+}
+
 struct XentGeom {
   int64_t n_rows_all, n_loss_rows, seq, ld;
 };
@@ -1170,8 +1206,8 @@
   return dx;
 }
 
-std::tuple<at::Tensor, at::Tensor> pool_bn_fwd(const at::Tensor& y, const at::Tensor& scale, const at::Tensor& shift,
-                                               int64_t p) {
+std::tuple<at::Tensor, at::Tensor, at::Tensor> pool_bn_fwd_impl(const at::Tensor& y, const at::Tensor& scale,
+                                                                const at::Tensor& shift, int64_t p, bool want_yarg) {
   check_dev(y, "y");
   TORCH_CHECK(y.dim() == 4 && y.is_contiguous(at::MemoryFormat::ChannelsLast) && y.scalar_type() == at::kBFloat16,
               "pool_bn: bf16 NHWC 4-D input");
@@ -1185,10 +1221,52 @@
   at::hip::HIPGuardMasqueradingAsCUDA guard(y.device());
   at::Tensor out = at::empty({N, C, Ho, Wo}, y.options().memory_format(at::MemoryFormat::ChannelsLast));
   at::Tensor arg = at::empty({N * Ho * Wo * C}, y.options().dtype(at::kByte));
+  at::Tensor yarg = want_yarg ? at::empty_like(out) : at::Tensor();
   check(madnn_pool_bn_fwd(y.data_ptr(), scale.data_ptr<float>(), shift.data_ptr<float>(), out.data_ptr(),
-                          arg.data_ptr(), (int)N, (int)H, (int)W, (int)C, (int)Ho, (int)Wo, (int)p, cur_stream(y)),
+                          arg.data_ptr(), want_yarg ? yarg.data_ptr() : nullptr, (int)N, (int)H, (int)W, (int)C,
+                          (int)Ho, (int)Wo, (int)p, cur_stream(y)),
         "pool_bn_fwd");
+  return {out, arg, yarg};
+}
+
+std::tuple<at::Tensor, at::Tensor> pool_bn_fwd(const at::Tensor& y, const at::Tensor& scale, const at::Tensor& shift,
+                                               int64_t p) {
+  auto [out, arg, yarg] = pool_bn_fwd_impl(y, scale, shift, p, false);
   return {out, arg};
+}
+
+std::tuple<at::Tensor, at::Tensor, at::Tensor> pool_bn_fwd_yarg(const at::Tensor& y, const at::Tensor& scale,
+                                                                const at::Tensor& shift, int64_t p) {
+  return pool_bn_fwd_impl(y, scale, shift, p, true);
+}
+
+std::tuple<at::Tensor, at::Tensor, at::Tensor> pool_bn_bwd_coef(const at::Tensor& dp, const at::Tensor& yarg,
+                                                                const c10::optional<at::Tensor>& w,
+                                                                const at::Tensor& mean, const at::Tensor& invstd,
+                                                                const at::Tensor& scale, const at::Tensor& shift,
+                                                                int64_t pixels) {
+  check_dev(dp, "dp");
+  check_dev(yarg, "yarg");
+  TORCH_CHECK(yarg.dim() == 4 && yarg.scalar_type() == at::kBFloat16 &&
+                  yarg.is_contiguous(at::MemoryFormat::ChannelsLast) && dp.sizes() == yarg.sizes() &&
+                  dp.strides() == yarg.strides() && dp.scalar_type() == at::kBFloat16,
+              "pool_bn_bwd_coef: dp and yarg must be channels_last bf16 of one shape");
+  const int64_t C = yarg.size(1), pooled = yarg.numel() / C;
+  TORCH_CHECK(madnn_pool_bn_supported(yarg.numel(), (int)C) && pooled > 0 && pixels > 0,
+              "pool_bn_bwd_coef: unsupported shape");
+  const float* sc = vec_ptr(scale, C, "pool_bn_bwd_coef", "scale");
+  const float* sh = vec_ptr(shift, C, "pool_bn_bwd_coef", "shift");
+  const float* mu = vec_ptr(mean, C, "pool_bn_bwd_coef", "mean");
+  const float* is = vec_ptr(invstd, C, "pool_bn_bwd_coef", "invstd");
+  at::hip::HIPGuardMasqueradingAsCUDA guard(yarg.device());
+  auto fo = yarg.options().dtype(at::kFloat);
+  at::Tensor dw = at::empty({C}, fo), db = at::empty({C}, fo), coef = at::empty({3, C}, fo);
+  at::Tensor ws = at::empty({(int64_t)madnn_pool_bn_bwd_pooled_rows(pooled, (int)C) * 2 * C}, fo);
+  check(madnn_pool_bn_bwd_pooled(dp.data_ptr(), yarg.data_ptr(), optf(w), mu, is, sc, sh, dw.data_ptr<float>(),
+                                 db.data_ptr<float>(), coef.data_ptr<float>(), ws.data_ptr<float>(), pooled, pixels,
+                                 (int)C, cur_stream(yarg)),
+        "pool_bn_bwd_coef");
+  return {coef, dw, db};
 }
 
 std::tuple<at::Tensor, at::Tensor, at::Tensor> pool_bn_bwd(const at::Tensor& dp, const at::Tensor& arg,
@@ -1515,6 +1593,9 @@
   m.def("conv3x3_fwd_s2(Tensor x, Tensor w, bool stats) -> (Tensor, Tensor)");
   m.def("conv3x3_wgrad(Tensor dy, Tensor x, bool out_bf16) -> Tensor");
   m.def("stem_wgrad(Tensor dy, Tensor x) -> Tensor");
+  m.def(
+      "stem_wgrad_bnp(Tensor x, Tensor y, Tensor dp, Tensor arg, Tensor scale, Tensor shift, Tensor coef, int p) -> "
+      "Tensor");
   m.def("bias_grad(Tensor dy, Tensor? pre, ScalarType bias_dtype, int gelu_kind=1) -> (Tensor, Tensor)");
   m.def("gelu_fwd(Tensor x, int kind=1) -> Tensor");
   m.def("rope_qkv_(Tensor(a!) qkv, Tensor cos, Tensor sin, int rot_heads, bool inverse) -> Tensor(a!)");
@@ -1523,6 +1604,10 @@
   m.def("swiglu_bwd(Tensor dh, Tensor gu) -> Tensor");
   m.def("maxpool_fwd(Tensor x, int k, int s, int p, bool need_arg) -> (Tensor, Tensor)");
   m.def("pool_bn_fwd(Tensor y, Tensor scale, Tensor shift, int p) -> (Tensor, Tensor)");
+  m.def("pool_bn_fwd_yarg(Tensor y, Tensor scale, Tensor shift, int p) -> (Tensor, Tensor, Tensor)");
+  m.def(
+      "pool_bn_bwd_coef(Tensor dp, Tensor yarg, Tensor? w, Tensor mean, Tensor invstd, Tensor scale, Tensor shift, "
+      "int pixels) -> (Tensor, Tensor, Tensor)");
   m.def(
       "pool_bn_bwd(Tensor dp, Tensor arg, Tensor y, Tensor? w, Tensor mean, Tensor invstd, Tensor scale, Tensor shift, "
       "int p) -> (Tensor, Tensor, Tensor)");
@@ -1567,6 +1652,8 @@
   m.impl("xent_rescale", xent_rescale);
   m.impl("maxpool_fwd", maxpool_fwd);
   m.impl("pool_bn_fwd", pool_bn_fwd);
+  m.impl("pool_bn_fwd_yarg", pool_bn_fwd_yarg);
+  m.impl("pool_bn_bwd_coef", pool_bn_bwd_coef);
   m.impl("pool_bn_bwd", pool_bn_bwd);
   m.impl("bias_grad", bias_grad);
   m.impl("gelu_fwd", gelu_fwd);
@@ -1585,6 +1672,7 @@
   m.impl("bn3_conv3_bwd", bn3_conv3_bwd);
   m.impl("stem_fwd", stem_fwd);
   m.impl("stem_wgrad", stem_wgrad);
+  m.impl("stem_wgrad_bnp", stem_wgrad_bnp);
   m.impl("linear_fwd", linear_fwd);
   m.impl("linear_dgrad", linear_dgrad);
   m.impl("linear_wgrad", linear_wgrad);
diff --git a/madnn/ops/csrc/pool.hip b/madnn/ops/csrc/pool.hip
--- a/madnn/ops/csrc/pool.hip
+++ b/madnn/ops/csrc/pool.hip
@@ -93,12 +93,14 @@
   return (blockIdx.x % kNumXCD) * (gridDim.x / kNumXCD) + blockIdx.x / kNumXCD;
 }
 
-template <int XDT, bool BNRELU = false>
+template <int XDT, bool BNRELU = false, bool YARG = false>
 __global__ __launch_bounds__(256) void maxpool_k3s2_fwd_kernel(const void* __restrict__ x, void* __restrict__ y,
                                                                uint64_t* __restrict__ arg, int N, int H, int W,
                                                                int C, int Ho, int Wo, int p, int swz,
                                                                const float* __restrict__ sc = nullptr,
-                                                               const float* __restrict__ sh = nullptr) {
+                                                               const float* __restrict__ sh = nullptr,
+                                                               void* __restrict__ yarg = nullptr) {
+  static_assert(!YARG || BNRELU, "yarg is the fused stem pool's");
   const unsigned CG = (unsigned)C >> 3;
   const unsigned total = (unsigned)N * Ho * Wo * CG;
   for (unsigned idx = xcd_block_id(swz) * blockDim.x + threadIdx.x; idx < total; idx += gridDim.x * blockDim.x) {
@@ -128,7 +130,7 @@
         }
       }
     }
-    if constexpr (BNRELU) {
+    if constexpr (BNRELU && !YARG) {
 #pragma unroll
       for (int q = 0; q < 9; ++q) {
         if (!ok[q]) continue;
@@ -139,7 +141,7 @@
         }
       }
     }
-    float best[8];
+    float best[8], raw[8];
     unsigned char a[8];
     unsigned char first = 0;
 #pragma unroll
@@ -148,6 +150,7 @@
 #pragma unroll
     for (int j = 0; j < 8; ++j) {
       best[j] = -__builtin_inff();
+      raw[j] = 0.f;
       a[j] = first;
     }
 #pragma unroll
@@ -155,13 +158,20 @@
       if (!ok[q]) continue;
 #pragma unroll
       for (int j = 0; j < 8; ++j) {
-        if (v[q][j] > best[j] || __builtin_isnan(v[q][j])) {
-          best[j] = v[q][j];
+        float t = v[q][j];
+        if constexpr (YARG) {
+          const float z = t * bs[j] + bh[j];
+          t = z > 0.f ? z : 0.f;
+        }
+        if (t > best[j] || __builtin_isnan(t)) {
+          best[j] = t;
           a[j] = (unsigned char)q;
+          if constexpr (YARG) raw[j] = v[q][j];
         }
       }
     }
     store8<XDT>(y, (int64_t)pix * C + cg * 8, best);
+    if constexpr (YARG) store8<XDT>(yarg, (int64_t)pix * C + cg * 8, raw);
     if (arg) {
       uint64_t packed = 0;
 #pragma unroll
@@ -312,6 +322,61 @@
   }
 }
 
+__global__ __launch_bounds__(256) void pool_bn_bwd_pooled_sums_kernel(const void* __restrict__ dp,
+                                                                      const void* __restrict__ yarg,
+                                                                      const float* __restrict__ sc,
+                                                                      const float* __restrict__ sh,
+                                                                      float* __restrict__ partial, unsigned total,
+                                                                      int C) {
+  __shared__ float slab[256][17];
+  const unsigned CG = (unsigned)C >> 3;
+  const unsigned cg = threadIdx.x % CG;
+  float bs[8], bh[8], s0[8], s1[8];
+  load8<kF32>(sc, cg * 8, bs);
+  load8<kF32>(sh, cg * 8, bh);
+#pragma unroll
+  for (int j = 0; j < 8; ++j) s0[j] = s1[j] = 0.f;
+  auto add = [&](const float (&g)[8], const float (&yv)[8]) {
+#pragma unroll
+    for (int j = 0; j < 8; ++j) {
+      const float z = yv[j] * bs[j] + bh[j];
+      const float gm = z > 0.f ? g[j] : 0.f;
+      s0[j] += gm;
+      s1[j] += gm * yv[j];
+    }
+  };
+  const unsigned stride = gridDim.x * blockDim.x;
+  unsigned idx = blockIdx.x * blockDim.x + threadIdx.x;
+  for (; idx + 3 * stride < total; idx += 4 * stride) {
+    float g[4][8], yv[4][8];
+#pragma unroll
+    for (int u = 0; u < 4; ++u) {
+      load8<kBF16>(dp, (int64_t)(idx + u * stride) * 8, g[u]);
+      load8<kBF16>(yarg, (int64_t)(idx + u * stride) * 8, yv[u]);
+    }
+#pragma unroll
+    for (int u = 0; u < 4; ++u) add(g[u], yv[u]);
+  }
+  for (; idx < total; idx += stride) {
+    float g[8], yv[8];
+    load8<kBF16>(dp, (int64_t)idx * 8, g);
+    load8<kBF16>(yarg, (int64_t)idx * 8, yv);
+    add(g, yv);
+  }
+#pragma unroll
+  for (int j = 0; j < 8; ++j) {
+    slab[threadIdx.x][j] = s0[j];
+    slab[threadIdx.x][8 + j] = s1[j];
+  }
+  __syncthreads();
+  for (int c = threadIdx.x; c < 2 * C; c += blockDim.x) {
+    const int which = c / C, ch = c % C, g8 = ch >> 3, e = ch & 7;
+    float a = 0.f;
+    for (int r = g8; r < 256; r += (int)CG) a += slab[r][which * 8 + e];
+    partial[(int64_t)blockIdx.x * 2 * C + c] = a;
+  }
+}
+
 }
 
 using namespace madnn;
@@ -382,13 +447,18 @@
   return numel < (1ll << 31) && C % 8 == 0 && C <= 2048 && 256 % (C / 8) == 0;
 }
 
-hipError_t madnn_pool_bn_fwd(const void* x, const float* scale, const float* shift, void* y, void* arg, int N, int H,
-                             int W, int C, int Ho, int Wo, int p, hipStream_t stream) {
+hipError_t madnn_pool_bn_fwd(const void* x, const float* scale, const float* shift, void* y, void* arg, void* yarg,
+                             int N, int H, int W, int C, int Ho, int Wo, int p, hipStream_t stream) {
   if (!madnn_pool_bn_supported((int64_t)N * H * W * C, C) || p > 2) return hipErrorInvalidValue;
   const int64_t work = (int64_t)N * Ho * Wo * (C / 8);
   const int grid = stream_grid(work, 256, g_pool_bn_wg[0] * kNumCU);
-  hipLaunchKernelGGL((maxpool_k3s2_fwd_kernel<kBF16, true>), dim3(grid), dim3(256), 0, stream, x, y,
-                     static_cast<uint64_t*>(arg), N, H, W, C, Ho, Wo, p, 0, scale, shift);
+  if (yarg) {
+    hipLaunchKernelGGL((maxpool_k3s2_fwd_kernel<kBF16, true, true>), dim3(grid), dim3(256), 0, stream, x, y,
+                       static_cast<uint64_t*>(arg), N, H, W, C, Ho, Wo, p, 0, scale, shift, yarg);
+  } else {
+    hipLaunchKernelGGL((maxpool_k3s2_fwd_kernel<kBF16, true>), dim3(grid), dim3(256), 0, stream, x, y,
+                       static_cast<uint64_t*>(arg), N, H, W, C, Ho, Wo, p, 0, scale, shift, nullptr);
+  }
   return hipGetLastError();
 }
 
@@ -420,4 +490,19 @@
   return hipGetLastError();
 }
 
-}
+int madnn_pool_bn_bwd_pooled_rows(int64_t pooled, int C) { return stream_grid(pooled * (C / 8), 256, 8 * kNumCU); }
+
+hipError_t madnn_pool_bn_bwd_pooled(const void* dp, const void* yarg, const float* w, const float* mean,
+                                    const float* invstd, const float* scale, const float* shift, float* dw, float* db,
+                                    float* coef, float* workspace, int64_t pooled, int64_t pixels, int C,
+                                    hipStream_t stream) {
+  if (!madnn_pool_bn_supported(pooled * C, C) || pooled <= 0) return hipErrorInvalidValue;
+  const int G = madnn_pool_bn_bwd_pooled_rows(pooled, C);
+  hipLaunchKernelGGL(pool_bn_bwd_pooled_sums_kernel, dim3(G), dim3(256), 0, stream, dp, yarg, scale, shift, workspace,
+                     (unsigned)(pooled * (C / 8)), C);
+  MADNN_HIP_CHECK(hipGetLastError());
+  return madnn_bn_bwd_finalize(workspace, G, C, 2 * C, C, pixels, w, mean, invstd, dw, db, coef, coef + C,
+                               coef + 2 * C, stream);
+}
+
+}
diff --git a/madnn/ops/csrc/stem.hip b/madnn/ops/csrc/stem.hip
--- a/madnn/ops/csrc/stem.hip
+++ b/madnn/ops/csrc/stem.hip
@@ -180,6 +180,15 @@
   float* ws;
   int N, H, W, Ho, Wo;
   int rows, per;
+  const uint16_t* y;
+  const uint16_t* dp;
+  const uint64_t* arg;
+  const float* sc;
+  const float* sh;
+  const float* ca;
+  const float* cb;
+  const float* cc;
+  int Hp, Wp, p;
 };
 
 __device__ __forceinline__ bf16x8 lds_patch(const uint16_t* img_row, int ow0, int lane) {
@@ -194,13 +203,19 @@
   return __builtin_bit_cast(bf16x8, r);
 }
 
+template <bool BNP>
 __global__ __launch_bounds__(kThreads, 2) void stem_wgrad_kernel(const StemWArgs a) {
   extern __shared__ __attribute__((aligned(16))) uint16_t smem[];
   const int WOP = (a.Wo + 15) & ~15;
   const int ROW = (2 * WOP + 6) * 4;
   uint16_t* ring = smem;
   uint16_t* dyt = smem + 9 * ROW;
-  const int tid = threadIdx.x, wave = tid >> 6, lane = tid & 63, hh = lane >> 5, l32 = lane & 31;
+  const int pchunks = BNP ? a.Wp * 8 : 0;
+  uint16_t* pdp = dyt + WOP * kCo;
+  uint64_t* parg = reinterpret_cast<uint64_t*>(pdp + 2 * pchunks * 8);
+  float* cf = reinterpret_cast<float*>(parg + 2 * pchunks);
+  int tid = threadIdx.x;
+  const int wave = tid >> 6, lane = tid & 63, hh = lane >> 5, l32 = lane & 31;
   const int row_elems = a.W * 3, chunks = row_elems / 8;
   const int dchunks = a.Wo * 8;
 
@@ -216,11 +231,45 @@
 
   u32x4 istg[4], dstg[4];
   int s_oh = 0, s_klo = 0;
+  u32x4 pstg[2];
+  u32x2 astg[2];
+  int s_pslot = -1;
+  auto pload = [&](int n, int ohp) {
+    if constexpr (BNP) asm volatile("" : "+v"(tid));
+    s_pslot = ohp & 1;
+    const int64_t base = ((int64_t)n * a.Hp + ohp) * pchunks;
+#pragma unroll
+    for (int i = 0; i < 2; ++i) {
+      const int c = tid + kThreads * i;
+      if (c < pchunks) {
+        pstg[i] = *reinterpret_cast<const u32x4*>(a.dp + (base + c) * 8);
+        astg[i] = *reinterpret_cast<const u32x2*>(a.arg + base + c);
+      }
+    }
+  };
+  auto pstore = [&]() {
+    if (s_pslot < 0) return;
+    if constexpr (BNP) asm volatile("" : "+v"(tid));
+#pragma unroll
+    for (int i = 0; i < 2; ++i) {
+      const int c = tid + kThreads * i;
+      if (c < pchunks) {
+        *reinterpret_cast<u32x4*>(pdp + (s_pslot * pchunks + c) * 8) = pstg[i];
+        *reinterpret_cast<u32x2*>(parg + s_pslot * pchunks + c) = astg[i];
+      }
+    }
+  };
   auto load = [&](int r) {
+    if constexpr (BNP) asm volatile("" : "+v"(tid));
     const int n = r / a.Ho, oh = r % a.Ho;
     const bool fresh = (r == r0) || (oh == 0);
     s_oh = oh;
     s_klo = fresh ? 0 : 5;
+    if constexpr (BNP) {
+      const int h1 = (oh + a.p) >> 1;
+      s_pslot = -1;
+      if ((fresh || ((oh + a.p) & 1) == 0) && h1 < a.Hp) pload(n, h1);
+    }
     const int total = (kKh - s_klo) * chunks;
 #pragma unroll
     for (int i = 0; i < 4; ++i) {
@@ -232,10 +281,12 @@
           istg[i] = *reinterpret_cast<const u32x4*>(a.x + ((int64_t)n * a.H + ih) * row_elems + (c % chunks) * 8);
       }
       const int d = tid + kThreads * i;
-      if (d < dchunks) dstg[i] = *reinterpret_cast<const u32x4*>(a.dy + ((int64_t)r * a.Wo) * kCo + d * 8);
+      if (d < dchunks)
+        dstg[i] = *reinterpret_cast<const u32x4*>((BNP ? a.y : a.dy) + ((int64_t)r * a.Wo) * kCo + d * 8);
     }
   };
   auto store = [&]() {
+    if constexpr (BNP) asm volatile("" : "+v"(tid));
     const int total = (kKh - s_klo) * chunks;
 #pragma unroll
     for (int i = 0; i < 4; ++i) {
@@ -251,16 +302,95 @@
           }
         }
       }
+      if constexpr (!BNP) {
+        const int d = tid + kThreads * i;
+        if (d < dchunks)
+          *reinterpret_cast<u32x4*>(reinterpret_cast<char*>(dyt) + swz<64>(d >> 3, d & 7)) = dstg[i];
+      }
+    }
+    if constexpr (BNP) pstore();
+  };
+  auto build = [&]() {
+    const int hp = s_oh + a.p, h1 = hp >> 1, hodd = hp & 1;
+    const bool okh[2] = {hodd == 0 && h1 >= 1, h1 < a.Hp};
+    if constexpr (BNP) asm volatile("" : "+v"(tid));
+    const int cg = tid & 7;
+    float v[5][8];
+#pragma unroll
+    for (int k = 0; k < 5; ++k) {
+      const f32x4 lo = *reinterpret_cast<const f32x4*>(cf + k * kCo + cg * 8);
+      const f32x4 hi = *reinterpret_cast<const f32x4*>(cf + k * kCo + cg * 8 + 4);
+      v[k][0] = lo.x; v[k][1] = lo.y; v[k][2] = lo.z; v[k][3] = lo.w;
+      v[k][4] = hi.x; v[k][5] = hi.y; v[k][6] = hi.z; v[k][7] = hi.w;
+    }
+#pragma unroll
+    for (int i = 0; i < 4; ++i) {
       const int d = tid + kThreads * i;
-      if (d < dchunks)
-        *reinterpret_cast<u32x4*>(reinterpret_cast<char*>(dyt) + swz<64>(d >> 3, d & 7)) = dstg[i];
-    }
-  };
-
+      if (d < dchunks) {
+        const int wp = (d >> 3) + a.p, w1 = wp >> 1, wodd = wp & 1;
+        const bool okw[2] = {wodd == 0 && w1 >= 1, w1 < a.Wp};
+        u32x4 g[4];
+        u32x2 pk[4];
+        bool ok[4];
+        unsigned pos[4];
+#pragma unroll
+        for (int q = 0; q < 4; ++q) {
+          const int ih = q >> 1, iw = q & 1;
+          ok[q] = okh[ih] && okw[iw];
+          pos[q] = (unsigned)((ih ? hodd : 2) * 3 + (iw ? wodd : 2));
+          const int ow = min(max(w1 - 1 + iw, 0), a.Wp - 1);
+          const int c = (((h1 - 1 + ih) & 1) * a.Wp + ow) * 8 + cg;
+          g[q] = *reinterpret_cast<const u32x4*>(pdp + c * 8);
+          pk[q] = *reinterpret_cast<const u32x2*>(parg + c);
+        }
+        u32x4 o4;
+#pragma unroll
+        for (int j2 = 0; j2 < 4; ++j2) {
+          unsigned short ob[2];
+#pragma unroll
+          for (int e = 0; e < 2; ++e) {
+            const int j = 2 * j2 + e;
+            float acc = 0.f;
+#pragma unroll
+            for (int q = 0; q < 4; ++q) {
+              const float gj = bf16_to_f32((unsigned short)((g[q][j >> 1] >> (16 * (j & 1))) & 0xffffu));
+              const unsigned byte = (pk[q][j >> 2] >> (8 * (j & 3))) & 0xffu;
+              if (ok[q]) acc += (byte == pos[q]) ? gj : 0.f;
+            }
+            const float yv = bf16_to_f32((unsigned short)((dstg[i][j >> 1] >> (16 * (j & 1))) & 0xffffu));
+            const float z = yv * v[0][j] + v[1][j];
+            acc = z > 0.f ? acc : 0.f;
+            ob[e] = f32_to_bf16(v[2][j] * acc + v[3][j] * yv + v[4][j]);
+          }
+          o4[j2] = (unsigned)ob[0] | ((unsigned)ob[1] << 16);
+        }
+        *reinterpret_cast<u32x4*>(reinterpret_cast<char*>(dyt) + swz<64>(d >> 3, d & 7)) = o4;
+      }
+      __builtin_amdgcn_sched_barrier(0);
+    }
+  };
+
+  if constexpr (BNP) {
+    for (int i = tid; i < 5 * kCo; i += kThreads) {
+      const float* src = i < kCo ? a.sc : i < 2 * kCo ? a.sh : i < 3 * kCo ? a.ca : i < 4 * kCo ? a.cb : a.cc;
+      cf[i] = src[i % kCo];
+    }
+  }
   __syncthreads();
+  if constexpr (BNP) {
+    const int n = r0 / a.Ho, hp = r0 % a.Ho + a.p;
+    if ((hp & 1) == 0 && (hp >> 1) >= 1) {
+      pload(n, (hp >> 1) - 1);
+      pstore();
+    }
+  }
   load(r0);
   store();
   __syncthreads();
+  if constexpr (BNP) {
+    build();
+    __syncthreads();
+  }
   for (int r = r0;;) {
     const int oh = r % a.Ho;
     const bool more = r + 1 < r1;
@@ -281,6 +411,10 @@
     __syncthreads();
     store();
     __syncthreads();
+    if constexpr (BNP) {
+      build();
+      __syncthreads();
+    }
     ++r;
   }
 
@@ -392,10 +526,47 @@
   const int grid = (a.rows + a.per - 1) / a.per;
   const int WOP = (a.Wo + 15) & ~15;
   const size_t lds = (size_t)(9 * (2 * WOP + 6) * 4 + WOP * kCo) * sizeof(uint16_t);
-  hipLaunchKernelGGL(stem_wgrad_kernel, dim3(grid), dim3(kThreads), lds, s, a);
+  hipLaunchKernelGGL(stem_wgrad_kernel<false>, dim3(grid), dim3(kThreads), lds, s, a);
   MADNN_HIP_CHECK(hipGetLastError());
   hipLaunchKernelGGL(stem_wgrad_reduce, dim3((kCo * 147 + 31) / 32), dim3(256), 0, s, ws, dw, grid);
   return hipGetLastError();
 }
 
-}
+hipError_t madnn_stem_wgrad_bnp(const void* x, const void* y, const void* dp, const void* arg, const float* scale,
+                                const float* shift, const float* ca, const float* cb, const float* cc, float* ws,
+                                float* dw, int N, int H, int W, int p, hipStream_t s) {
+  if (!madnn_stem_supported(H, W) || p < 0 || p > 1) return hipErrorInvalidValue;
+  StemWArgs a{};
+  a.x = static_cast<const uint16_t*>(x);
+  a.y = static_cast<const uint16_t*>(y);
+  a.dp = static_cast<const uint16_t*>(dp);
+  a.arg = static_cast<const uint64_t*>(arg);
+  a.sc = scale;
+  a.sh = shift;
+  a.ca = ca;
+  a.cb = cb;
+  a.cc = cc;
+  a.ws = ws;
+  a.N = N;
+  a.H = H;
+  a.W = W;
+  a.Ho = (H + 6 - 7) / 2 + 1;
+  a.Wo = (W + 6 - 7) / 2 + 1;
+  a.p = p;
+  a.Hp = (a.Ho + 2 * p - 3) / 2 + 1;
+  a.Wp = (a.Wo + 2 * p - 3) / 2 + 1;
+  if (a.Ho + 2 * p < 3 || a.Wo + 2 * p < 3) return hipErrorInvalidValue;
+  a.rows = N * a.Ho;
+  if (a.rows <= 0) return hipMemsetAsync(dw, 0, sizeof(float) * kCo * 147, s);
+  a.per = (a.rows + wgrad_grid(a.rows) - 1) / wgrad_grid(a.rows);
+  const int grid = (a.rows + a.per - 1) / a.per;
+  const int WOP = (a.Wo + 15) & ~15;
+  const size_t lds = (size_t)(9 * (2 * WOP + 6) * 4 + WOP * kCo) * sizeof(uint16_t) + (size_t)2 * a.Wp * kCo * 3 +
+                     5 * kCo * sizeof(float);
+  hipLaunchKernelGGL(stem_wgrad_kernel<true>, dim3(grid), dim3(kThreads), lds, s, a);
+  MADNN_HIP_CHECK(hipGetLastError());
+  hipLaunchKernelGGL(stem_wgrad_reduce, dim3((kCo * 147 + 31) / 32), dim3(256), 0, s, ws, dw, grid);
+  return hipGetLastError();
+}
+
+}
```

New measurement: 14110, median of 6. 1.01x the previous value.
